# abstractqqq/polars_ds_extension

Hardware: AMD Instinct MI355X
Metric: grouped lstsq regressions/sec (1e8 rows x 16 f64 feats; Gram-build GB/s under gram_build) (higher is better)
Workload: dtype f64; 1 GPU; group_by(key).agg(lin_reg): 1000000 groups x 100 rows x 16 f64 feats of the frame (1e+08 rows), OLS with rank gate (pl_lr default path), inputs resident in HBM; `value`: the groups given as row offsets (pre-segmented, as Polars hands groups to pl_lr -- the cpu_baseline gets the same); the same step starting from a sorted int64 key column: grouped_by_key; groups_total=1000000, groups_per_gpu=1000000, rows_per_group=100, features=16, parallelism=group-sharded x1

## Files before the change

polars_ds_extension_amd/_lib.py:

```python
from __future__ import annotations

import ctypes as C
from pathlib import Path

_HERE = Path(__file__).resolve().parent
LIB_PATH = _HERE / "csrc" / "libpds_lstsq_hip.so"

PDS_HOST, PDS_DEVICE = 0, 1
SOLVERS = {"qr": 0, "svd": 1, "choleskey": 2}
SE_TYPES = {"se": 0, "hc0": 1, "hc1": 2, "hc2": 3, "hc3": 4}
WITHIN_SE_TYPES = {"se": 0, "cluster": 5, "cluster0": 6}
CLUSTER_SE_TYPES = {"cluster": 5, "cluster0": 6}
GLM_ROBUST_SE_TYPES = {"hc0": 1, "hc1": 2, "hc2": 3, "hc3": 4, "cluster": 5, "cluster0": 6}
PDS_REPORT_DERIVE_YVAR = 0x100

EXPORTS = [
    "pds_last_error", "pds_version", "pds_ctx_create", "pds_ctx_destroy", "pds_ctx_set_stream",
    "pds_ctx_synchronize", "pds_ctx_num_cus", "pds_ctx_set_option", "pds_ctx_get_option", "pds_grouped_fused_split", "pds_set_host_staging", "pds_rows_to_cols_f64", "pds_rows_to_cols_f32", "pds_glm_irls_f64", "pds_glm_irls_f32", "pds_glm_irls_grouped_f64", "pds_glm_irls_grouped_f32", "pds_glm_irls_by_key_f64", "pds_glm_irls_by_key_f32",
    "pds_glm_irls_wo_f64", "pds_glm_irls_wo_f32", "pds_glm_irls_wo_grouped_f64", "pds_glm_irls_wo_grouped_f32", "pds_glm_irls_wo_by_key_f64", "pds_glm_irls_wo_by_key_f32",
    "pds_glm_enet_f64", "pds_glm_enet_f32", "pds_glm_enet_grouped_f64", "pds_glm_enet_grouped_f32", "pds_glm_enet_by_key_f64", "pds_glm_enet_by_key_f32",
    "pds_glm_report_wo_grouped_f64", "pds_glm_report_wo_grouped_f32", "pds_glm_report_wo_by_key_f64", "pds_glm_report_wo_by_key_f32",
    "pds_glm_report_grouped_f64", "pds_glm_report_grouped_f32", "pds_glm_report_by_key_f64", "pds_glm_report_by_key_f32",
    "pds_glm_report_robust_f64", "pds_glm_report_robust_f32", "pds_glm_report_cluster_grouped_f64", "pds_glm_report_cluster_grouped_f32",
    "pds_glm_report_cluster_by_key_f64", "pds_glm_report_cluster_by_key_f32",
# ... 21 lines not shown
    "pds_lr_grouped_f64", "pds_lr_grouped_f32",
    "pds_rolling_lr_f64", "pds_rolling_lr_f32", "pds_recursive_lr_f64", "pds_recursive_lr_f32",
    "pds_recursive_lr_seeded_f64", "pds_recursive_lr_seeded_f32",
    "pds_rolling_lr_grouped_f64", "pds_rolling_lr_grouped_f32", "pds_recursive_lr_grouped_f64", "pds_recursive_lr_grouped_f32",
    "pds_rolling_lr_by_key_f64", "pds_rolling_lr_by_key_f32", "pds_recursive_lr_by_key_f64", "pds_recursive_lr_by_key_f32",
    "pds_lin_reg_report_nullable_f64", "pds_lin_reg_report_nullable_f32",
    "pds_lr_grouped_nullable_f64", "pds_lr_grouped_nullable_f32",
    "pds_lr_by_key_f64", "pds_lr_by_key_f32", "pds_lr_by_key_multi_f64", "pds_lr_by_key_multi_f32", "pds_lr_by_key_pred_multi_f64", "pds_lr_by_key_pred_multi_f32", "pds_host_alloc", "pds_host_free", "pds_device_count", "pds_device_alloc", "pds_device_free", "pds_ipc_export", "pds_ipc_open", "pds_ipc_close", "pds_signal_post", "pds_signal_wait", "pds_signal_wait_status", "pds_lr_grouped_pred_f64", "pds_lr_grouped_pred_f32", "pds_lr_by_key_pred_f64", "pds_lr_by_key_pred_f32", "pds_lr_grouped_weighted_f64", "pds_lr_grouped_weighted_f32",
    "pds_lr_with_inv_f64", "pds_lr_with_inv_f32",
    "pds_moments_f64", "pds_moments_f32", "pds_lr_from_moments_f64", "pds_lr_from_moments_f32",
    "pds_student_t_sf", "pds_student_t_ppf",
    "pds_allreduce_sum_f64", "pds_allreduce_sum_f32", "pds_scatter_rows_f64", "pds_scatter_rows_f32", "pds_gather_f64", "pds_gather_f32",
]


class LRParams(C.Structure):

    _fields_ = [
        ("add_bias", C.c_int),
        ("l1_reg", C.c_double),
        ("l2_reg", C.c_double),
        ("tol", C.c_double),
        ("solver", C.c_int),
        ("positive", C.c_int),
        ("max_iter", C.c_int),
        ("singular_x_tol", C.c_double),
    ]


class ReportF64(C.Structure):
    _fields_ = [(k, C.c_void_p) for k in ("beta", "std_err", "t", "p", "ci_lower", "ci_upper")] + [
        ("r2", C.c_double),
        ("adj_r2", C.c_double),
    ]


class ReportF32(C.Structure):
    _fields_ = [(k, C.c_void_p) for k in ("beta", "std_err", "t", "p", "ci_lower", "ci_upper")] + [
        ("r2", C.c_float),
        ("adj_r2", C.c_float),
    ]


class ReportGrouped(C.Structure):
    _fields_ = [(k, C.c_void_p) for k in ("beta", "std_err", "t", "p", "ci_lower", "ci_upper", "r2", "adj_r2", "is_null")]


class GlmReportOut(C.Structure):
    _fields_ = [(k, C.c_void_p) for k in ("std_err", "z", "p", "ci_lower", "ci_upper", "cov", "deviance", "null_deviance", "pearson_chi2",
                                          "dispersion", "df_resid", "report_null")]


class WithinOut(C.Structure):
    _fields_ = [("alpha", C.c_void_p), ("pred", C.c_void_p), ("resid", C.c_void_p), ("r2_overall", C.c_double),
                ("n_groups_used", C.c_int64), ("df_resid", C.c_int64)]


class GlmWithinOut(C.Structure):
    _fields_ = [(k, C.c_double * 16) for k in ("beta", "std_err", "z", "p", "ci_lower", "ci_upper")] + [
        ("cov", C.c_double * 256), ("deviance", C.c_double), ("pearson_chi2", C.c_double), ("dispersion", C.c_double),
        ("n_groups_used", C.c_int64), ("n_groups_dropped", C.c_int64), ("n_rows_used", C.c_int64), ("df_resid", C.c_int64),
        ("n_iter", C.c_int32), ("converged", C.c_int32), ("alpha", C.c_void_p), ("pred", C.c_void_p)]


class Within2Out(C.Structure):
    _fields_ = [("pred", C.c_void_p), ("resid", C.c_void_p), ("r2_overall", C.c_double), ("df_resid", C.c_int64),
                ("n_groups_used", C.c_int64), ("n_groups2_used", C.c_int64), ("n_components", C.c_int64), ("n_iter", C.c_int64)]


class Within2Effects(C.Structure):
    _fields_ = [("effects1", C.c_void_p), ("effects2", C.c_void_p), ("component1", C.c_void_p), ("component2", C.c_void_p),
                ("keys1", C.c_void_p), ("cap1", C.c_int64), ("n_graph_rounds", C.c_int64)]


class ClusterKey(C.Structure):
    _fields_ = [("codes", C.c_void_p), ("n_levels", C.c_int64), ("n_clusters", C.c_int64), ("nested1", C.c_int32), ("nested2", C.c_int32)]


class PdsError(RuntimeError):
    def __init__(self, code: int, msg: str):
        super().__init__(f"[pds {code}] {msg}")
        self.code = code
        self.msg = msg


_lib = None


def load() -> C.CDLL:
    global _lib
    if _lib is None:
        if not LIB_PATH.exists():
            raise ImportError(
                f"{LIB_PATH} is missing: run `python -c 'import __graft_entry__ as g; g.build()'` "
                "(hipcc --offload-arch=gfx950).  There is no CPU fallback."
            )
        try:
            import torch
        except Exception:
            pass
        lib = C.CDLL(str(LIB_PATH))
        lib.pds_last_error.restype = C.c_char_p
        lib.pds_version.restype = C.c_char_p
        lib.pds_student_t_sf.restype = C.c_double
        lib.pds_student_t_sf.argtypes = [C.c_double, C.c_double]
        lib.pds_student_t_ppf.restype = C.c_double
        lib.pds_student_t_ppf.argtypes = [C.c_double, C.c_double]
        lib.pds_ctx_create.argtypes = [C.c_int, C.POINTER(C.c_void_p)]
        lib.pds_ctx_destroy.argtypes = [C.c_void_p]
        lib.pds_ctx_destroy.restype = None
        lib.pds_ctx_set_stream.argtypes = [C.c_void_p, C.c_void_p]
        lib.pds_ctx_synchronize.argtypes = [C.c_void_p]
        lib.pds_ctx_num_cus.argtypes = [C.c_void_p]
        lib.pds_ctx_set_option.argtypes = [C.c_void_p, C.c_char_p, C.c_longlong]
        if hasattr(lib, "pds_ctx_get_option"):
            lib.pds_ctx_get_option.argtypes = [C.c_void_p, C.c_char_p, C.POINTER(C.c_longlong)]
        if hasattr(lib, "pds_set_host_staging"):
            lib.pds_set_host_staging.argtypes = [C.c_double, C.c_double]
        if hasattr(lib, "pds_ctx_workspace_spills"):
            lib.pds_ctx_workspace_spills.argtypes = [C.c_void_p]
            lib.pds_ctx_workspace_spills.restype = C.c_longlong
        for sfx, real in (("f64", C.c_double), ("f32", C.c_float)):
            if hasattr(lib, "pds_lr_multi_grouped_" + sfx):
                getattr(lib, "pds_lr_multi_grouped_" + sfx).argtypes = [C.c_void_p, C.c_void_p, C.c_int, C.c_int, C.c_int64, C.c_void_p,
                                                                      C.c_int64, C.c_int, C.c_int, real, C.c_int, real] + [C.c_void_p] * 5
                getattr(lib, "pds_lr_multi_by_key_" + sfx).argtypes = [C.c_void_p, C.c_void_p, C.c_void_p, C.c_int, C.c_int, C.c_int64, C.c_int,
                                                                     C.c_int, real, C.c_int, real, C.c_int64] + [C.c_void_p] * 7
            if hasattr(lib, "pds_lin_reg_within_grouped_" + sfx):
                getattr(lib, "pds_lin_reg_within_grouped_" + sfx).argtypes = [C.c_void_p, C.c_void_p, C.c_int, C.c_int64, C.c_void_p, C.c_int64,
                                                                            C.c_int, C.c_int, C.c_void_p, C.c_void_p]
                getattr(lib, "pds_lin_reg_within_by_key_" + sfx).argtypes = [C.c_void_p, C.c_void_p, C.c_void_p, C.c_int, C.c_int64, C.c_int, C.c_int,
                                                                           C.c_int64, C.c_void_p, C.c_void_p, C.c_void_p, C.c_void_p]
            if hasattr(lib, "pds_lin_reg_within2_grouped_" + sfx):
                getattr(lib, "pds_lin_reg_within2_grouped_" + sfx).argtypes = [C.c_void_p, C.c_void_p, C.c_int, C.c_int64, C.c_void_p, C.c_int64,
                                                                             C.c_void_p, C.c_int64, C.c_int, C.c_int, C.c_double, C.c_int,
                                                                             C.c_void_p, C.c_void_p]
                getattr(lib, "pds_lin_reg_within2_by_key_" + sfx).argtypes = [C.c_void_p, C.c_void_p, C.c_void_p, C.c_void_p, C.c_int64, C.c_int,
                                                                            C.c_int64, C.c_int, C.c_int, C.c_double, C.c_int, C.c_void_p,
                                                                            C.c_void_p, C.c_void_p]
            if hasattr(lib, "pds_lin_reg_within2_fx_grouped_" + sfx):
                getattr(lib, "pds_lin_reg_within2_fx_grouped_" + sfx).argtypes = getattr(lib, "pds_lin_reg_within2_grouped_" + sfx).argtypes + [C.c_void_p]
                getattr(lib, "pds_lin_reg_within2_fx_by_key_" + sfx).argtypes = getattr(lib, "pds_lin_reg_within2_by_key_" + sfx).argtypes + [C.c_void_p]
            if hasattr(lib, "pds_lin_reg_within_cl_grouped_" + sfx):
                for form in ("grouped_", "by_key_"):
                    getattr(lib, "pds_lin_reg_within_cl_" + form + sfx).argtypes = getattr(lib, "pds_lin_reg_within_" + form + sfx).argtypes + [C.c_void_p]
                    getattr(lib, "pds_lin_reg_within2_cl_" + form + sfx).argtypes = getattr(lib, "pds_lin_reg_within2_fx_" + form + sfx).argtypes + [C.c_void_p]
            if hasattr(lib, "pds_glm_within_grouped_" + sfx):
                getattr(lib, "pds_glm_within_grouped_" + sfx).argtypes = [C.c_void_p] * 4 + [C.c_int, C.c_int64, C.c_void_p, C.c_int64, C.c_int,
                                                                                             C.c_int, C.c_int, real, C.c_int, C.c_int, C.c_void_p]
                getattr(lib, "pds_glm_within_by_key_" + sfx).argtypes = [C.c_void_p] * 5 + [C.c_int, C.c_int64, C.c_int, C.c_int, C.c_int, real,
                                                                                            C.c_int, C.c_int, C.c_int64] + [C.c_void_p] * 3
        if hasattr(lib, "pds_absorb_components_i32"):
            lib.pds_absorb_components_i32.argtypes = [C.c_void_p, C.c_void_p, C.c_int64, C.c_void_p, C.c_int64, C.c_int64, C.c_int] + [C.c_void_p] * 6
        if hasattr(lib, "pds_ctx_workspace_bytes"):
            lib.pds_ctx_workspace_bytes.argtypes = [C.c_void_p, C.c_int]
            lib.pds_ctx_workspace_bytes.restype = C.c_longlong
        _lib = lib
    return _lib


def check(rc: int) -> None:
    if rc != 0:
        raise PdsError(rc, load().pds_last_error().decode("utf-8", "replace"))


def missing_exports() -> list[str]:
    lib = load()
    return [s for s in EXPORTS if not hasattr(lib, s)]
```

polars_ds_extension_amd/csrc/capi.hip:

```cpp
#include <algorithm>
#include <atomic>
#include <condition_variable>
#include <mutex>
#include <thread>
#include <chrono>
#include <cstdio>
#include <cstdlib>
#include <mutex>

#include <hipcub/hipcub.hpp>

#include "common.hpp"
#include "grouped_report.hpp"
#include "grouped_split_dev.hpp"

namespace pds {

#include "capi_core.hpp"
#include "capi_staging.hpp"
#include "capi_lr.hpp"
#include "capi_report.hpp"
#include "capi_staged_out.hpp"
#include "capi_keyed_frame.hpp"
#include "capi_group_chunks.hpp"
#include "capi_grouped.hpp"
#include "capi_report_grouped.hpp"
#include "capi_multi.hpp"
#include "capi_rolling.hpp"
#include "capi_models.hpp"
#include "capi_glm_grouped.hpp"
#include "capi_glm_report.hpp"
#include "capi_rcond_grouped.hpp"
#include "capi_multi_grouped.hpp"
#include "capi_mixed.hpp"
#include "capi_report_cluster.hpp"
#include "capi_within_cluster.hpp"
#include "capi_within.hpp"
#include "capi_within2.hpp"
#include "capi_glm_sandwich.hpp"
#include "capi_glm_within.hpp"

}

using namespace pds;

template <typename F>
static int with_cluster_key(pds_cluster_key* cl, pds_space space, F&& call) {
    if (!cl) return call(nullptr);
    pds::WithinCluster wc;
    wc.codes = cl->codes;
    wc.code_space = space;
    wc.n_levels = cl->n_levels;
    const int rc = call(&wc);
    cl->n_clusters = wc.n_clusters;
    cl->nested1 = wc.nested1;
    cl->nested2 = wc.nested2;
    return rc;
}

extern "C" {

const char* pds_last_error(void) { return g_err.c_str(); }
const char* pds_version(void) { return "pds_lstsq_hip 0.1.0 (gfx950)"; }

int pds_ctx_create(int device, pds_ctx** out) {
    if (!out) return fail(PDS_ERR_INVALID, "null out pointer");
    int ndev = 0;
    PDS_HIP_CHECK(hipGetDeviceCount(&ndev));
    if (device < 0 || device >= ndev) return fail(PDS_ERR_HIP, "no such HIP device");
    hipDeviceProp_t prop;
    PDS_HIP_CHECK(hipGetDeviceProperties(&prop, device));
    if (std::string(prop.gcnArchName).rfind("gfx950", 0) != 0)
        return fail(PDS_ERR_HIP, std::string("libpds_lstsq_hip is built for gfx950 only, device is ") + prop.gcnArchName);
    PDS_HIP_CHECK(hipSetDevice(device));
    pds_ctx* c = new pds_ctx();
    c->device = device;
    c->num_cus = prop.multiProcessorCount;
    if (hipStreamCreateWithFlags(&c->stream, hipStreamNonBlocking) != hipSuccess) {
        delete c;
        return fail(PDS_ERR_HIP, "hipStreamCreate failed");
    }
    c->own_stream = true;
    {
        const char* ks = std::getenv("PDS_KEYED_SORT");
        c->opt_keyed_sort = ks && ks[0] == '1';
        const char* wn = std::getenv("PDS_WIDE_F32_NATIVE");
        c->opt_wide_f32_native = wn && wn[0] == '1';
    }
    const size_t pbytes = (size_t)c->num_cus * 8 * kPartStride * sizeof(double);
    if (hipMalloc(reinterpret_cast<void**>(&c->partials), pbytes) != hipSuccess) {
        (void)hipStreamDestroy(c->stream);
        delete c;
        return fail(PDS_ERR_HIP, "hipMalloc(partials) failed");
    }
    *out = c;
    return PDS_OK;
}

void pds_ctx_destroy(pds_ctx* ctx) {
    if (!ctx) return;
    (void)hipSetDevice(ctx->device);
    (void)hipStreamSynchronize(ctx->stream);
    if (ctx->partials) (void)hipFree(ctx->partials);
    if (ctx->ws.ptr) (void)hipFree(ctx->ws.ptr);
    for (void* q : ctx->ws_spill) (void)hipFree(q);
    if (ctx->stage.ptr) (void)hipFree(ctx->stage.ptr);
    if (ctx->solve_ws.ptr) (void)hipFree(ctx->solve_ws.ptr);
    if (ctx->keyed.ptr) (void)hipFree(ctx->keyed.ptr);
    if (ctx->wkeyed.ptr) (void)hipFree(ctx->wkeyed.ptr);
    if (ctx->mark_count) (void)hipFree(ctx->mark_count);
    if (ctx->wait_timeouts) (void)hipFree(ctx->wait_timeouts);
    if (ctx->mark_host) (void)hipHostFree(ctx->mark_host);
    if (ctx->pinned) (void)hipHostFree(ctx->pinned);
    if (ctx->pinned_in) (void)hipHostFree(ctx->pinned_in);
    for (auto& e : ctx->ev_pending) {
        (void)hipEventDestroy(e.a);
        (void)hipEventDestroy(e.b);
    }
    for (auto e : ctx->ev_pool) (void)hipEventDestroy(e);
    if (ctx->own_stream && ctx->stream) (void)hipStreamDestroy(ctx->stream);
    delete ctx;
}

int pds_ctx_set_stream(pds_ctx* ctx, void* hip_stream) {
    if (!ctx) return fail(PDS_ERR_INVALID, "null ctx");
    PDS_HIP_CHECK(hipSetDevice(ctx->device));
    PDS_HIP_CHECK(hipStreamSynchronize(ctx->stream));
    if (ctx->own_stream && ctx->stream) (void)hipStreamDestroy(ctx->stream);
    ctx->stream = reinterpret_cast<hipStream_t>(hip_stream);
    ctx->own_stream = false;
    return PDS_OK;
}

int pds_ctx_synchronize(pds_ctx* ctx) {
    if (!ctx) return fail(PDS_ERR_INVALID, "null ctx");
    PDS_HIP_CHECK(hipStreamSynchronize(ctx->stream));
    return PDS_OK;
}

int pds_ctx_num_cus(const pds_ctx* ctx) { return ctx ? ctx->num_cus : 0; }

int pds_ctx_set_option(pds_ctx* ctx, const char* name, long long value) {
    if (!ctx || !name) return fail(PDS_ERR_INVALID, "null argument");
    const std::string n(name);
    if (n == "keyed_sort") ctx->opt_keyed_sort = value != 0;
    else if (n == "wide_f32_native") ctx->opt_wide_f32_native = value != 0;
    else if (n == "glm_split_rows") ctx->opt_glm_split_rows = value > 0 ? (int64_t)value : 0;
    else if (n == "mixed_split_rows") ctx->opt_mixed_split_rows = value > 0 ? (int64_t)value : 0;
    else if (n == "cluster_split_rows") ctx->opt_cluster_split_rows = value > 0 ? (int64_t)value : 0;
    else if (n == "cluster_waves") ctx->opt_cluster_waves = value > 0 ? (int64_t)value : 0;
    else if (n == "within_split_rows") ctx->opt_within_split_rows = value > 0 ? (int64_t)value : 0;
    else if (n == "within2_accel") {
        if (value != 0 && value != 1) return fail(PDS_ERR_INVALID, "within2_accel: 0 (plain sweeps) or 1 (Irons-Tuck)");
        ctx->opt_within2_accel = (int64_t)value;
    } else if (n == "report_chunk_groups") ctx->opt_report_chunk_groups = value > 0 ? (int64_t)value : 0;
    else if (n == "grouped_fused_waves") ctx->opt_fused_waves = value > 0 ? (int64_t)value : 0;
    else if (n == "grouped_fused_late_permille") {
        if (value < 0 || value > 999) return fail(PDS_ERR_INVALID, "grouped_fused_late_permille: 0 (the default rule) or 1 .. 999");
        ctx->opt_fused_late_permille = (int64_t)value;
    } else if (n == "grouped_multi_route") {
        if (value < 0 || value > 2) return fail(PDS_ERR_INVALID, "grouped_multi_route: 0 (choose), 1 (one kernel) or 2 (per target)");
        ctx->opt_multi_route = (int64_t)value;
    } else if (n == "grouped_multi_waves") ctx->opt_multi_waves = value > 0 ? (int64_t)value : 0;
    else if (n == "rolling_waves") ctx->opt_rolling_waves = value > 0 ? (int64_t)value : 0;
    else return fail(PDS_ERR_INVALID, "unknown context option: " + n);
    return PDS_OK;
}

int pds_ctx_get_option(const pds_ctx* ctx, const char* name, long long* value) {
    if (!ctx || !name || !value) return fail(PDS_ERR_INVALID, "null argument");
    const std::string n(name);
    if (n == "keyed_sort") *value = ctx->opt_keyed_sort ? 1 : 0;
    else if (n == "wide_f32_native") *value = ctx->opt_wide_f32_native ? 1 : 0;
    else if (n == "glm_split_rows") *value = ctx->opt_glm_split_rows;
    else if (n == "mixed_split_rows") *value = ctx->opt_mixed_split_rows;
    else if (n == "cluster_split_rows") *value = ctx->opt_cluster_split_rows;
    else if (n == "cluster_waves") *value = ctx->opt_cluster_waves;
    else if (n == "within_split_rows") *value = ctx->opt_within_split_rows;
    else if (n == "within2_accel") *value = ctx->opt_within2_accel;
    else if (n == "report_chunk_groups") *value = ctx->opt_report_chunk_groups;
    else if (n == "grouped_fused_waves") *value = ctx->opt_fused_waves;
    else if (n == "grouped_fused_late_permille") *value = ctx->opt_fused_late_permille;
    else if (n == "grouped_multi_route") *value = ctx->opt_multi_route;
    else if (n == "grouped_multi_waves") *value = ctx->opt_multi_waves;
    else if (n == "rolling_waves") *value = ctx->opt_rolling_waves;
    else return fail(PDS_ERR_INVALID, "unknown context option: " + n);
    return PDS_OK;
}

int pds_grouped_fused_split(const int64_t* group_offsets, int64_t n_groups, int waves, int late_permille, int64_t* first_group,
                            int64_t* end_group) {
    if (!group_offsets || !first_group || !end_group) return fail(PDS_ERR_INVALID, "null argument");
    if (n_groups < 0 || waves < 1 || late_permille < 0 || late_permille > 999) return fail(PDS_ERR_INVALID, "pds_grouped_fused_split: bad argument");
    const int64_t base = group_offsets[0], total = group_offsets[n_groups] - base;
    auto bound = [&](int64_t w) -> int64_t {
        if (w == 0) return 0;
        if (w == waves) return n_groups;
        return std::lower_bound(group_offsets, group_offsets + n_groups, base + pds::fused_split_row(w, waves, total, late_permille)) - group_offsets;
    };
    for (int w = 0; w < waves; ++w) {
        first_group[w] = bound(w);
        end_group[w] = std::max(bound(w + 1), first_group[w]);
    }
    return PDS_OK;
}

int pds_glm_irls_f64(pds_ctx* ctx, const double* const* cols, int n_feat, int64_t n_rows, pds_space space, int add_bias, int link,
                     int variance, double tol, int max_iter, double* coeffs, int* n_iter) {
    return pds::glm_irls_impl<double>(ctx, cols, n_feat, n_rows, space, add_bias, link, variance, tol, max_iter, coeffs, n_iter);
}
int pds_glm_irls_f32(pds_ctx* ctx, const float* const* cols, int n_feat, int64_t n_rows, pds_space space, int add_bias, int link,
                     int variance, float tol, int max_iter, float* coeffs, int* n_iter) {
    return pds::glm_irls_impl<float>(ctx, cols, n_feat, n_rows, space, add_bias, link, variance, tol, max_iter, coeffs, n_iter);
}

int pds_glm_irls_grouped_f64(pds_ctx* ctx, const double* const* cols, int n_feat, int64_t n_rows, const int64_t* group_offsets,
                             int64_t n_groups, pds_space space, int add_bias, int link, int variance, double tol, int max_iter,
                             double* coeffs, int32_t* n_iter, uint8_t* is_null, double* pred, uint8_t* row_null) {
    return pds::glm_grouped_impl<double>(ctx, cols, n_feat, n_rows, group_offsets, n_groups, space, add_bias, link, variance, 0.0, 0.0, tol,
                                         max_iter, coeffs, n_iter, is_null, pred, row_null);
}
int pds_glm_irls_grouped_f32(pds_ctx* ctx, const float* const* cols, int n_feat, int64_t n_rows, const int64_t* group_offsets,
                             int64_t n_groups, pds_space space, int add_bias, int link, int variance, float tol, int max_iter,
                             float* coeffs, int32_t* n_iter, uint8_t* is_null, float* pred, uint8_t* row_null) {
    return pds::glm_grouped_impl<float>(ctx, cols, n_feat, n_rows, group_offsets, n_groups, space, add_bias, link, variance, 0.0f, 0.0f, tol,
                                        max_iter, coeffs, n_iter, is_null, pred, row_null);
}
int pds_glm_irls_by_key_f64(pds_ctx* ctx, const double* const* cols, const int64_t* keys, int n_feat, int64_t n_rows, pds_space space,
                            int add_bias, int link, int variance, double tol, int max_iter, int64_t max_groups, int64_t* out_keys,
                            double* coeffs, int32_t* n_iter, uint8_t* is_null, int64_t* n_groups, double* pred, uint8_t* row_null) {
    return pds::glm_by_key_impl<double>(ctx, cols, keys, n_feat, n_rows, space, add_bias, link, variance, 0.0, 0.0, tol, max_iter, max_groups,
                                        out_keys, coeffs, n_iter, is_null, n_groups, pred, row_null);
}
int pds_glm_irls_by_key_f32(pds_ctx* ctx, const float* const* cols, const int64_t* keys, int n_feat, int64_t n_rows, pds_space space,
                            int add_bias, int link, int variance, float tol, int max_iter, int64_t max_groups, int64_t* out_keys,
                            float* coeffs, int32_t* n_iter, uint8_t* is_null, int64_t* n_groups, float* pred, uint8_t* row_null) {
    return pds::glm_by_key_impl<float>(ctx, cols, keys, n_feat, n_rows, space, add_bias, link, variance, 0.0f, 0.0f, tol, max_iter, max_groups,
                                       out_keys, coeffs, n_iter, is_null, n_groups, pred, row_null);
}

int pds_glm_irls_wo_f64(pds_ctx* ctx, const double* const* cols, const double* weights, const double* offset, int n_feat, int64_t n_rows,
                        pds_space space, int add_bias, int link, int variance, double tol, int max_iter, double* coeffs, int* n_iter) {
    return pds::glm_irls_wo_impl<double>(ctx, cols, weights, offset, n_feat, n_rows, space, add_bias, link, variance, tol, max_iter, coeffs,
                                         n_iter);
}
int pds_glm_irls_wo_f32(pds_ctx* ctx, const float* const* cols, const float* weights, const float* offset, int n_feat, int64_t n_rows,
                        pds_space space, int add_bias, int link, int variance, float tol, int max_iter, float* coeffs, int* n_iter) {
    return pds::glm_irls_wo_impl<float>(ctx, cols, weights, offset, n_feat, n_rows, space, add_bias, link, variance, tol, max_iter, coeffs,
                                        n_iter);
}
int pds_glm_irls_wo_grouped_f64(pds_ctx* ctx, const double* const* cols, const double* weights, const double* offset, int n_feat,
                                int64_t n_rows, const int64_t* group_offsets, int64_t n_groups, pds_space space, int add_bias, int link,
                                int variance, double tol, int max_iter, double* coeffs, int32_t* n_iter, uint8_t* is_null, double* pred,
                                uint8_t* row_null) {
    return pds::glm_grouped_impl<double>(ctx, cols, n_feat, n_rows, group_offsets, n_groups, space, add_bias, link, variance, 0.0, 0.0, tol,
                                         max_iter, coeffs, n_iter, is_null, pred, row_null, nullptr, weights, offset);
}
int pds_glm_irls_wo_grouped_f32(pds_ctx* ctx, const float* const* cols, const float* weights, const float* offset, int n_feat, int64_t n_rows,
                                const int64_t* group_offsets, int64_t n_groups, pds_space space, int add_bias, int link, int variance,
                                float tol, int max_iter, float* coeffs, int32_t* n_iter, uint8_t* is_null, float* pred, uint8_t* row_null) {
    return pds::glm_grouped_impl<float>(ctx, cols, n_feat, n_rows, group_offsets, n_groups, space, add_bias, link, variance, 0.0f, 0.0f, tol,
                                        max_iter, coeffs, n_iter, is_null, pred, row_null, nullptr, weights, offset);
}
int pds_glm_irls_wo_by_key_f64(pds_ctx* ctx, const double* const* cols, const double* weights, const double* offset, const int64_t* keys,
                               int n_feat, int64_t n_rows, pds_space space, int add_bias, int link, int variance, double tol, int max_iter,
                               int64_t max_groups, int64_t* out_keys, double* coeffs, int32_t* n_iter, uint8_t* is_null, int64_t* n_groups,
                               double* pred, uint8_t* row_null) {
    return pds::glm_by_key_impl<double>(ctx, cols, keys, n_feat, n_rows, space, add_bias, link, variance, 0.0, 0.0, tol, max_iter, max_groups,
                                        out_keys, coeffs, n_iter, is_null, n_groups, pred, row_null, weights, offset);
}
int pds_glm_irls_wo_by_key_f32(pds_ctx* ctx, const float* const* cols, const float* weights, const float* offset, const int64_t* keys,
                               int n_feat, int64_t n_rows, pds_space space, int add_bias, int link, int variance, float tol, int max_iter,
                               int64_t max_groups, int64_t* out_keys, float* coeffs, int32_t* n_iter, uint8_t* is_null, int64_t* n_groups,
                               float* pred, uint8_t* row_null) {
    return pds::glm_by_key_impl<float>(ctx, cols, keys, n_feat, n_rows, space, add_bias, link, variance, 0.0f, 0.0f, tol, max_iter, max_groups,
                                       out_keys, coeffs, n_iter, is_null, n_groups, pred, row_null, weights, offset);
}

int pds_glm_report_grouped_f64(pds_ctx* ctx, const double* const* cols, int n_feat, int64_t n_rows, const int64_t* group_offsets,
                               int64_t n_groups, pds_space space, int add_bias, int link, int variance, double tol, int max_iter,
                               double* coeffs, int32_t* n_iter, uint8_t* is_null, const pds_glm_report_out* out) {
    return pds::glm_report_grouped_impl<double>(ctx, cols, n_feat, n_rows, group_offsets, n_groups, space, add_bias, link, variance, tol,
                                                max_iter, coeffs, n_iter, is_null, out);
}
int pds_glm_report_grouped_f32(pds_ctx* ctx, const float* const* cols, int n_feat, int64_t n_rows, const int64_t* group_offsets,
                               int64_t n_groups, pds_space space, int add_bias, int link, int variance, float tol, int max_iter,
                               float* coeffs, int32_t* n_iter, uint8_t* is_null, const pds_glm_report_out* out) {
    return pds::glm_report_grouped_impl<float>(ctx, cols, n_feat, n_rows, group_offsets, n_groups, space, add_bias, link, variance, tol,
                                               max_iter, coeffs, n_iter, is_null, out);
}
int pds_glm_report_by_key_f64(pds_ctx* ctx, const double* const* cols, const int64_t* keys, int n_feat, int64_t n_rows, pds_space space,
                              int add_bias, int link, int variance, double tol, int max_iter, int64_t max_groups, int64_t* out_keys,
                              double* coeffs, int32_t* n_iter, uint8_t* is_null, int64_t* n_groups, const pds_glm_report_out* out) {
    return pds::glm_report_by_key_impl<double>(ctx, cols, keys, n_feat, n_rows, space, add_bias, link, variance, tol, max_iter, max_groups,
                                               out_keys, coeffs, n_iter, is_null, n_groups, out);
}
int pds_glm_report_by_key_f32(pds_ctx* ctx, const float* const* cols, const int64_t* keys, int n_feat, int64_t n_rows, pds_space space,
                              int add_bias, int link, int variance, float tol, int max_iter, int64_t max_groups, int64_t* out_keys,
                              float* coeffs, int32_t* n_iter, uint8_t* is_null, int64_t* n_groups, const pds_glm_report_out* out) {
    return pds::glm_report_by_key_impl<float>(ctx, cols, keys, n_feat, n_rows, space, add_bias, link, variance, tol, max_iter, max_groups,
                                              out_keys, coeffs, n_iter, is_null, n_groups, out);
}

int pds_glm_report_wo_grouped_f64(pds_ctx* ctx, const double* const* cols, const double* weights, const double* offset, int n_feat, int64_t n_rows,
                                  const int64_t* group_offsets, int64_t n_groups, pds_space space, int add_bias, int link, int variance,
                                  double tol, int max_iter, double* coeffs, int32_t* n_iter, uint8_t* is_null, const pds_glm_report_out* out) {
    return pds::glm_report_grouped_impl<double>(ctx, cols, n_feat, n_rows, group_offsets, n_groups, space, add_bias, link, variance, tol,
                                                max_iter, coeffs, n_iter, is_null, out, weights, offset);
}
int pds_glm_report_wo_by_key_f64(pds_ctx* ctx, const double* const* cols, const double* weights, const double* offset, const int64_t* keys, int n_feat,
                                 int64_t n_rows, pds_space space, int add_bias, int link, int variance, double tol, int max_iter,
                                 int64_t max_groups, int64_t* out_keys, double* coeffs, int32_t* n_iter, uint8_t* is_null, int64_t* n_groups,
                                 const pds_glm_report_out* out) {
    return pds::glm_report_by_key_impl<double>(ctx, cols, keys, n_feat, n_rows, space, add_bias, link, variance, tol, max_iter, max_groups,
                                               out_keys, coeffs, n_iter, is_null, n_groups, out, weights, offset);
}
int pds_glm_report_wo_grouped_f32(pds_ctx* ctx, const float* const* cols, const float* weights, const float* offset, int n_feat, int64_t n_rows,
                                  const int64_t* group_offsets, int64_t n_groups, pds_space space, int add_bias, int link, int variance,
                                  float tol, int max_iter, float* coeffs, int32_t* n_iter, uint8_t* is_null, const pds_glm_report_out* out) {
    return pds::glm_report_grouped_impl<float>(ctx, cols, n_feat, n_rows, group_offsets, n_groups, space, add_bias, link, variance, tol,
                                                max_iter, coeffs, n_iter, is_null, out, weights, offset);
}
int pds_glm_report_wo_by_key_f32(pds_ctx* ctx, const float* const* cols, const float* weights, const float* offset, const int64_t* keys, int n_feat,
                                 int64_t n_rows, pds_space space, int add_bias, int link, int variance, float tol, int max_iter,
                                 int64_t max_groups, int64_t* out_keys, float* coeffs, int32_t* n_iter, uint8_t* is_null, int64_t* n_groups,
                                 const pds_glm_report_out* out) {
    return pds::glm_report_by_key_impl<float>(ctx, cols, keys, n_feat, n_rows, space, add_bias, link, variance, tol, max_iter, max_groups,
                                               out_keys, coeffs, n_iter, is_null, n_groups, out, weights, offset);
}

int pds_glm_report_robust_f64(pds_ctx* ctx, const double* const* cols, const double* weights, const double* offset, int n_feat, int64_t n_rows,
                              pds_space space, int add_bias, int link, int variance, double tol, int max_iter, int se_type, double* coeffs,
                              int32_t* n_iter, const pds_glm_report_out* out, int64_t* n_clusters) {
    return pds::glm_sandwich_impl<double>(ctx, cols, weights, offset, n_feat, n_rows, nullptr, 0, space, add_bias, link, variance, tol, max_iter,
                                       se_type, false, coeffs, n_iter, out, n_clusters);
}
int pds_glm_report_cluster_grouped_f64(pds_ctx* ctx, const double* const* cols, const double* weights, const double* offset, int n_feat,
                                       int64_t n_rows, const int64_t* cluster_offsets, int64_t n_offsets, pds_space space, int add_bias,
// ... 371 lines not shown
                                                absorb_tol, absorb_max_iter, out, extra);
}
int pds_lin_reg_within2_grouped_f32(pds_ctx* ctx, const float* const* cols, int n_feat, int64_t n_rows, const int64_t* group_offsets,
                                    int64_t n_groups, const int32_t* codes2, int64_t n_levels2, pds_space space, int se_type,
                                    double absorb_tol, int absorb_max_iter, pds_report_f32* out, pds_within2_out* extra) {
    return within2_impl<float, pds_report_f32>(ctx, cols, n_feat, n_rows, group_offsets, n_groups, space, codes2, space, n_levels2, space, se_type,
                                               absorb_tol, absorb_max_iter, out, extra);
}
int pds_lin_reg_within2_by_key_f64(pds_ctx* ctx, const double* const* cols, const int64_t* keys, const int32_t* codes2, int64_t n_levels2,
                                   int n_feat, int64_t n_rows, pds_space space, int se_type, double absorb_tol, int absorb_max_iter,
                                   pds_report_f64* out, pds_within2_out* extra, int64_t* n_groups) {
    return within2_by_key_impl<double, pds_report_f64>(ctx, cols, keys, codes2, n_levels2, n_feat, n_rows, space, se_type, absorb_tol,
                                                       absorb_max_iter, out, extra, n_groups);
}
int pds_lin_reg_within2_by_key_f32(pds_ctx* ctx, const float* const* cols, const int64_t* keys, const int32_t* codes2, int64_t n_levels2,
                                   int n_feat, int64_t n_rows, pds_space space, int se_type, double absorb_tol, int absorb_max_iter,
                                   pds_report_f32* out, pds_within2_out* extra, int64_t* n_groups) {
    return within2_by_key_impl<float, pds_report_f32>(ctx, cols, keys, codes2, n_levels2, n_feat, n_rows, space, se_type, absorb_tol,
                                                      absorb_max_iter, out, extra, n_groups);
}
int pds_lin_reg_within2_fx_grouped_f64(pds_ctx* ctx, const double* const* cols, int n_feat, int64_t n_rows, const int64_t* group_offsets,
                                       int64_t n_groups, const int32_t* codes2, int64_t n_levels2, pds_space space, int se_type,
                                       double absorb_tol, int absorb_max_iter, pds_report_f64* out, pds_within2_out* extra,
                                       pds_within2_effects* fx) {
    return within2_impl<double, pds_report_f64>(ctx, cols, n_feat, n_rows, group_offsets, n_groups, space, codes2, space, n_levels2, space, se_type,
                                                absorb_tol, absorb_max_iter, out, extra, nullptr, fx);
}
int pds_lin_reg_within2_fx_grouped_f32(pds_ctx* ctx, const float* const* cols, int n_feat, int64_t n_rows, const int64_t* group_offsets,
                                       int64_t n_groups, const int32_t* codes2, int64_t n_levels2, pds_space space, int se_type,
                                       double absorb_tol, int absorb_max_iter, pds_report_f32* out, pds_within2_out* extra,
                                       pds_within2_effects* fx) {
    return within2_impl<float, pds_report_f32>(ctx, cols, n_feat, n_rows, group_offsets, n_groups, space, codes2, space, n_levels2, space, se_type,
                                               absorb_tol, absorb_max_iter, out, extra, nullptr, fx);
}
int pds_lin_reg_within2_fx_by_key_f64(pds_ctx* ctx, const double* const* cols, const int64_t* keys, const int32_t* codes2, int64_t n_levels2,
                                      int n_feat, int64_t n_rows, pds_space space, int se_type, double absorb_tol, int absorb_max_iter,
                                      pds_report_f64* out, pds_within2_out* extra, int64_t* n_groups, pds_within2_effects* fx) {
    return within2_by_key_impl<double, pds_report_f64>(ctx, cols, keys, codes2, n_levels2, n_feat, n_rows, space, se_type, absorb_tol,
                                                       absorb_max_iter, out, extra, n_groups, fx);
}
int pds_lin_reg_within2_fx_by_key_f32(pds_ctx* ctx, const float* const* cols, const int64_t* keys, const int32_t* codes2, int64_t n_levels2,
                                      int n_feat, int64_t n_rows, pds_space space, int se_type, double absorb_tol, int absorb_max_iter,
                                      pds_report_f32* out, pds_within2_out* extra, int64_t* n_groups, pds_within2_effects* fx) {
    return within2_by_key_impl<float, pds_report_f32>(ctx, cols, keys, codes2, n_levels2, n_feat, n_rows, space, se_type, absorb_tol,
                                                      absorb_max_iter, out, extra, n_groups, fx);
}
int pds_lin_reg_within_cl_grouped_f64(pds_ctx* ctx, const double* const* cols, int n_feat, int64_t n_rows, const int64_t* group_offsets,
                                      int64_t n_groups, pds_space space, int se_type, pds_report_f64* out, pds_within_out* extra, pds_cluster_key* cl) {
    return with_cluster_key(cl, space, [&](WithinCluster* wc) {
        return within_impl<double, pds_report_f64>(ctx, cols, n_feat, n_rows, group_offsets, n_groups, space, space, se_type, out, extra, nullptr, nullptr, wc);
    });
}
int pds_lin_reg_within_cl_by_key_f64(pds_ctx* ctx, const double* const* cols, const int64_t* keys, int n_feat, int64_t n_rows, pds_space space,
                                     int se_type, int64_t max_groups, int64_t* out_keys, pds_report_f64* out, pds_within_out* extra, int64_t* n_groups,
                                     pds_cluster_key* cl) {
    return with_cluster_key(cl, space, [&](WithinCluster* wc) {
        return within_by_key_impl<double, pds_report_f64>(ctx, cols, keys, n_feat, n_rows, space, se_type, max_groups, out_keys, out, extra, n_groups, wc);
    });
}
int pds_lin_reg_within2_cl_grouped_f64(pds_ctx* ctx, const double* const* cols, int n_feat, int64_t n_rows, const int64_t* group_offsets,
                                       int64_t n_groups, const int32_t* codes2, int64_t n_levels2, pds_space space, int se_type,
                                       double absorb_tol, int absorb_max_iter, pds_report_f64* out, pds_within2_out* extra, pds_within2_effects* fx,
                                       pds_cluster_key* cl) {
    return with_cluster_key(cl, space, [&](WithinCluster* wc) {
        return within2_impl<double, pds_report_f64>(ctx, cols, n_feat, n_rows, group_offsets, n_groups, space, codes2, space, n_levels2, space, se_type, absorb_tol,
                                        absorb_max_iter, out, extra, nullptr, fx, wc);
    });
}
int pds_lin_reg_within2_cl_by_key_f64(pds_ctx* ctx, const double* const* cols, const int64_t* keys, const int32_t* codes2, int64_t n_levels2,
                                      int n_feat, int64_t n_rows, pds_space space, int se_type, double absorb_tol, int absorb_max_iter,
                                      pds_report_f64* out, pds_within2_out* extra, int64_t* n_groups, pds_within2_effects* fx, pds_cluster_key* cl) {
    return with_cluster_key(cl, space, [&](WithinCluster* wc) {
        return within2_by_key_impl<double, pds_report_f64>(ctx, cols, keys, codes2, n_levels2, n_feat, n_rows, space, se_type, absorb_tol, absorb_max_iter, out,
                                               extra, n_groups, fx, wc);
    });
}
int pds_lin_reg_within_cl_grouped_f32(pds_ctx* ctx, const float* const* cols, int n_feat, int64_t n_rows, const int64_t* group_offsets,
                                      int64_t n_groups, pds_space space, int se_type, pds_report_f32* out, pds_within_out* extra, pds_cluster_key* cl) {
    return with_cluster_key(cl, space, [&](WithinCluster* wc) {
        return within_impl<float, pds_report_f32>(ctx, cols, n_feat, n_rows, group_offsets, n_groups, space, space, se_type, out, extra, nullptr, nullptr, wc);
    });
}
int pds_lin_reg_within_cl_by_key_f32(pds_ctx* ctx, const float* const* cols, const int64_t* keys, int n_feat, int64_t n_rows, pds_space space,
                                     int se_type, int64_t max_groups, int64_t* out_keys, pds_report_f32* out, pds_within_out* extra, int64_t* n_groups,
                                     pds_cluster_key* cl) {
    return with_cluster_key(cl, space, [&](WithinCluster* wc) {
        return within_by_key_impl<float, pds_report_f32>(ctx, cols, keys, n_feat, n_rows, space, se_type, max_groups, out_keys, out, extra, n_groups, wc);
    });
}
int pds_lin_reg_within2_cl_grouped_f32(pds_ctx* ctx, const float* const* cols, int n_feat, int64_t n_rows, const int64_t* group_offsets,
                                       int64_t n_groups, const int32_t* codes2, int64_t n_levels2, pds_space space, int se_type,
                                       double absorb_tol, int absorb_max_iter, pds_report_f32* out, pds_within2_out* extra, pds_within2_effects* fx,
                                       pds_cluster_key* cl) {
    return with_cluster_key(cl, space, [&](WithinCluster* wc) {
        return within2_impl<float, pds_report_f32>(ctx, cols, n_feat, n_rows, group_offsets, n_groups, space, codes2, space, n_levels2, space, se_type, absorb_tol,
                                        absorb_max_iter, out, extra, nullptr, fx, wc);
    });
}
int pds_lin_reg_within2_cl_by_key_f32(pds_ctx* ctx, const float* const* cols, const int64_t* keys, const int32_t* codes2, int64_t n_levels2,
                                      int n_feat, int64_t n_rows, pds_space space, int se_type, double absorb_tol, int absorb_max_iter,
                                      pds_report_f32* out, pds_within2_out* extra, int64_t* n_groups, pds_within2_effects* fx, pds_cluster_key* cl) {
    return with_cluster_key(cl, space, [&](WithinCluster* wc) {
        return within2_by_key_impl<float, pds_report_f32>(ctx, cols, keys, codes2, n_levels2, n_feat, n_rows, space, se_type, absorb_tol, absorb_max_iter, out,
                                               extra, n_groups, fx, wc);
    });
}
int pds_absorb_components_i32(pds_ctx* ctx, const int32_t* codes1, int64_t n_levels1, const int32_t* codes2, int64_t n_levels2, int64_t n_rows,
                              pds_space space, int32_t* component1, int32_t* component2, int64_t* n1, int64_t* n2, int64_t* n_components,
                              int* n_rounds) {
    return absorb_components_impl(ctx, codes1, n_levels1, codes2, n_levels2, n_rows, space, component1, component2, n1, n2, n_components, n_rounds);
}

int pds_report_fit_from_moments_f64(pds_ctx* ctx, const double* moments, int n_feat, int add_bias, double* beta, double* inv) {
    return report_fit_impl<double>(ctx, moments, n_feat, add_bias, beta, inv);
}
int pds_report_fit_from_moments_f32(pds_ctx* ctx, const float* moments, int n_feat, int add_bias, float* beta, float* inv) {
    return report_fit_impl<float>(ctx, moments, n_feat, add_bias, beta, inv);
}
int pds_report_partials_f64(pds_ctx* ctx, const double* const* cols, const double* weights, int n_feat, int64_t n_rows,
                            pds_space space, int add_bias, int se_type, const double* beta, const double* inv, double* partials) {
    return report_partials_impl<double>(ctx, cols, weights, n_feat, n_rows, space, add_bias, se_type, beta, inv, partials);
}
int pds_report_partials_f32(pds_ctx* ctx, const float* const* cols, const float* weights, int n_feat, int64_t n_rows,
                            pds_space space, int add_bias, int se_type, const float* beta, const float* inv, double* partials) {
    return report_partials_impl<float>(ctx, cols, weights, n_feat, n_rows, space, add_bias, se_type, beta, inv, partials);
}
int pds_report_finish_f64(int n_feat, int add_bias, int se_type, int weighted, int64_t n_rows_total, double y_var,
                          const double* beta, const double* inv, const double* partials, pds_report_f64* out) {
    return report_finish_impl<double, pds_report_f64>(n_feat, add_bias, se_type, weighted, n_rows_total, y_var, beta, inv, partials, out);
}
int pds_report_finish_f32(int n_feat, int add_bias, int se_type, int weighted, int64_t n_rows_total, float y_var,
                          const float* beta, const float* inv, const double* partials, pds_report_f32* out) {
    return report_finish_impl<float, pds_report_f32>(n_feat, add_bias, se_type, weighted, n_rows_total, y_var, beta, inv, partials, out);
}

int pds_lin_reg_report_nullable_f64(pds_ctx* ctx, const double* const* cols, const uint8_t* const* validity,
                                    const int64_t* bit_offsets, int n_feat, int64_t n_rows, pds_space space, int null_policy,
                                    double fill_value, int add_bias, int se_type, double y_var, pds_report_f64* out,
                                    int64_t* n_used) {
    return report_impl<double, pds_report_f64>(ctx, cols, nullptr, n_feat, n_rows, space, add_bias, se_type, y_var, out, true,
                                               validity, bit_offsets, null_policy, fill_value, n_used);
}
int pds_lin_reg_report_nullable_f32(pds_ctx* ctx, const float* const* cols, const uint8_t* const* validity,
                                    const int64_t* bit_offsets, int n_feat, int64_t n_rows, pds_space space, int null_policy,
                                    float fill_value, int add_bias, int se_type, float y_var, pds_report_f32* out,
                                    int64_t* n_used) {
    return report_impl<float, pds_report_f32>(ctx, cols, nullptr, n_feat, n_rows, space, add_bias, se_type, y_var, out, true,
                                              validity, bit_offsets, null_policy, fill_value, n_used);
}

int pds_lr_grouped_f64(pds_ctx* ctx, const double* const* cols, int n_feat, int64_t n_rows,
                       const int64_t* group_offsets, int64_t n_groups, pds_space space, const pds_lr_params* prm,
                       double* coeffs, uint8_t* is_null) {
    return grouped_impl<double>(ctx, cols, n_feat, n_rows, group_offsets, n_groups, space, prm, coeffs, is_null);
}
int pds_lr_grouped_f32(pds_ctx* ctx, const float* const* cols, int n_feat, int64_t n_rows,
                       const int64_t* group_offsets, int64_t n_groups, pds_space space, const pds_lr_params* prm,
                       float* coeffs, uint8_t* is_null) {
    return grouped_impl<float>(ctx, cols, n_feat, n_rows, group_offsets, n_groups, space, prm, coeffs, is_null);
}

int pds_lr_grouped_nullable_f64(pds_ctx* ctx, const double* const* cols, const uint8_t* const* validity,
                                const int64_t* bit_offsets, int n_feat, int64_t n_rows, const int64_t* group_offsets,
                                int64_t n_groups, pds_space space, int null_policy, double fill_value, const pds_lr_params* prm,
                                double* coeffs, uint8_t* is_null) {
    return grouped_impl<double>(ctx, cols, n_feat, n_rows, group_offsets, n_groups, space, prm, coeffs, is_null, true, validity,
                                bit_offsets, null_policy, fill_value);
}
int pds_lr_grouped_nullable_f32(pds_ctx* ctx, const float* const* cols, const uint8_t* const* validity,
                                const int64_t* bit_offsets, int n_feat, int64_t n_rows, const int64_t* group_offsets,
                                int64_t n_groups, pds_space space, int null_policy, float fill_value, const pds_lr_params* prm,
                                float* coeffs, uint8_t* is_null) {
    return grouped_impl<float>(ctx, cols, n_feat, n_rows, group_offsets, n_groups, space, prm, coeffs, is_null, true, validity,
                               bit_offsets, null_policy, fill_value);
}

int pds_lr_with_inv_f64(pds_ctx* ctx, const double* const* cols, int n_feat, int64_t n_rows, pds_space space, int add_bias,
                        double lambda, double* coeffs, double* inv) {
    return pds::lr_with_inv_impl<double>(ctx, cols, n_feat, n_rows, space, add_bias, lambda, coeffs, inv);
}
int pds_lr_with_inv_f32(pds_ctx* ctx, const float* const* cols, int n_feat, int64_t n_rows, pds_space space, int add_bias,
                        float lambda, float* coeffs, float* inv) {
    return pds::lr_with_inv_impl<float>(ctx, cols, n_feat, n_rows, space, add_bias, (double)lambda, coeffs, inv);
}

int pds_lr_grouped_weighted_f64(pds_ctx* ctx, const double* const* cols, const double* weights, int n_feat, int64_t n_rows,
                                const int64_t* group_offsets, int64_t n_groups, pds_space space, const pds_lr_params* prm,
                                double* coeffs, uint8_t* is_null) {
    return pds::grouped_weighted_impl<double>(ctx, cols, weights, n_feat, n_rows, group_offsets, n_groups, space, prm, coeffs, is_null);
}
int pds_lr_grouped_weighted_f32(pds_ctx* ctx, const float* const* cols, const float* weights, int n_feat, int64_t n_rows,
                                const int64_t* group_offsets, int64_t n_groups, pds_space space, const pds_lr_params* prm,
                                float* coeffs, uint8_t* is_null) {
    return pds::grouped_weighted_impl<float>(ctx, cols, weights, n_feat, n_rows, group_offsets, n_groups, space, prm, coeffs, is_null);
}

int pds_lr_by_key_multi_f64(pds_ctx* const* ctxs, int n_ctx, int n_slices, const double* const* cols, const int64_t* keys, int n_feat,
                            int64_t n_rows, const pds_lr_params* prm, int64_t max_groups, int64_t* out_keys, double* coeffs,
                            uint8_t* is_null, int64_t* n_groups) {
    return pds::lr_by_key_multi_impl<double>(ctxs, n_ctx, n_slices, cols, keys, n_feat, n_rows, prm, max_groups, out_keys, coeffs, is_null,
                                             n_groups);
}
int pds_lr_by_key_multi_f32(pds_ctx* const* ctxs, int n_ctx, int n_slices, const float* const* cols, const int64_t* keys, int n_feat,
                            int64_t n_rows, const pds_lr_params* prm, int64_t max_groups, int64_t* out_keys, float* coeffs,
                            uint8_t* is_null, int64_t* n_groups) {
    return pds::lr_by_key_multi_impl<float>(ctxs, n_ctx, n_slices, cols, keys, n_feat, n_rows, prm, max_groups, out_keys, coeffs, is_null,
                                            n_groups);
}
int pds_lr_by_key_pred_multi_f64(pds_ctx* const* ctxs, int n_ctx, int n_slices, const double* const* cols, const double* weights,
                                 const int64_t* keys, int n_feat, int64_t n_rows, const pds_lr_params* prm, double* pred, double* resid,
                                 uint8_t* row_null) {
    return pds::lr_by_key_pred_multi_impl<double>(ctxs, n_ctx, n_slices, cols, weights, keys, n_feat, n_rows, prm, pred, resid, row_null);
}
int pds_lr_by_key_pred_multi_f32(pds_ctx* const* ctxs, int n_ctx, int n_slices, const float* const* cols, const float* weights,
                                 const int64_t* keys, int n_feat, int64_t n_rows, const pds_lr_params* prm, float* pred, float* resid,
                                 uint8_t* row_null) {
    return pds::lr_by_key_pred_multi_impl<float>(ctxs, n_ctx, n_slices, cols, weights, keys, n_feat, n_rows, prm, pred, resid, row_null);
}
int pds_host_alloc(size_t bytes, void** out) {
    if (!out) return pds::fail(PDS_ERR_INVALID, "null argument");
    *out = nullptr;
    PDS_HIP_CHECK(hipHostMalloc(out, bytes ? bytes : 1, hipHostMallocPortable));
    return PDS_OK;
}
int pds_host_free(void* p) {
    if (p) PDS_HIP_CHECK(hipHostFree(p));
    return PDS_OK;
}
int pds_device_count(int* n) {
    if (!n) return pds::fail(PDS_ERR_INVALID, "null argument");
    *n = 0;
    PDS_HIP_CHECK(hipGetDeviceCount(n));
    return PDS_OK;
}
static_assert(sizeof(hipIpcMemHandle_t) == PDS_IPC_HANDLE_BYTES, "the handle travels as 64 opaque bytes");
int pds_device_alloc(int device, size_t bytes, int fine_grained, void** out) {
    if (!out) return pds::fail(PDS_ERR_INVALID, "null argument");
    *out = nullptr;
    PDS_HIP_CHECK(hipSetDevice(device));
    if (fine_grained) PDS_HIP_CHECK(hipExtMallocWithFlags(out, bytes ? bytes : 1, hipDeviceMallocFinegrained));
    else PDS_HIP_CHECK(hipMalloc(out, bytes ? bytes : 1));
    return PDS_OK;
}
namespace pds {
__global__ void signal_post_kernel(unsigned* word, unsigned value) {
    __hip_atomic_store(word, value, __ATOMIC_RELEASE, __HIP_MEMORY_SCOPE_SYSTEM);
}
__global__ __launch_bounds__(64) void signal_wait_kernel(const unsigned* words, int n, unsigned value, long long budget_ticks, int* timed_out) {
    const int lane = threadIdx.x;
    const long long t0 = wall_clock64();
    bool ok = lane >= n;
    while (!__all(ok)) {
        if (!ok) ok = (int)(__hip_atomic_load(words + lane, __ATOMIC_ACQUIRE, __HIP_MEMORY_SCOPE_SYSTEM) - value) >= 0;
        if (wall_clock64() - t0 > budget_ticks) {
            if (lane == 0) atomicAdd(timed_out, 1);
            break;
        }
        __builtin_amdgcn_s_sleep(8);
    }
}
}
int pds_signal_post(pds_ctx* ctx, unsigned* word, unsigned value) {
    if (!ctx || !word) return pds::fail(PDS_ERR_INVALID, "null argument");
    PDS_HIP_CHECK(hipSetDevice(ctx->device));
    hipLaunchKernelGGL(pds::signal_post_kernel, dim3(1), dim3(1), 0, ctx->stream, word, value);
    PDS_HIP_CHECK(hipGetLastError());
    return PDS_OK;
}
int pds_signal_wait(pds_ctx* ctx, const unsigned* words, int n_words, unsigned value, int timeout_ms) {
    if (!ctx || !words || n_words < 0 || n_words > 64) return pds::fail(PDS_ERR_INVALID, "pds_signal_wait: up to 64 words");
    if (n_words == 0) return PDS_OK;
    PDS_HIP_CHECK(hipSetDevice(ctx->device));
    if (!ctx->wait_timeouts) {
        PDS_HIP_CHECK(hipMalloc(reinterpret_cast<void**>(&ctx->wait_timeouts), 64));
        PDS_HIP_CHECK(hipMemsetAsync(ctx->wait_timeouts, 0, 64, ctx->stream));
    }
    int rate_khz = 100000;
    (void)hipDeviceGetAttribute(&rate_khz, hipDeviceAttributeWallClockRate, ctx->device);
    const long long budget = (long long)(timeout_ms > 0 ? timeout_ms : 2000) * (long long)rate_khz;
    hipLaunchKernelGGL(pds::signal_wait_kernel, dim3(1), dim3(64), 0, ctx->stream, words, n_words, value, budget,
                       ctx->wait_timeouts);
    PDS_HIP_CHECK(hipGetLastError());
    return PDS_OK;
}
int pds_signal_wait_status(pds_ctx* ctx, int* timed_out) {
    if (!ctx || !timed_out) return pds::fail(PDS_ERR_INVALID, "null argument");
    *timed_out = 0;
    if (!ctx->wait_timeouts) return PDS_OK;
    PDS_HIP_CHECK(hipSetDevice(ctx->device));
    PDS_HIP_CHECK(hipMemcpyAsync(timed_out, ctx->wait_timeouts, sizeof(int), hipMemcpyDeviceToHost, ctx->stream));
    PDS_HIP_CHECK(hipStreamSynchronize(ctx->stream));
    return PDS_OK;
}
int pds_device_free(int device, void* p) {
    if (!p) return PDS_OK;
    PDS_HIP_CHECK(hipSetDevice(device));
    PDS_HIP_CHECK(hipFree(p));
    return PDS_OK;
}
int pds_ipc_export(int device, void* p, unsigned char* handle) {
    if (!p || !handle) return pds::fail(PDS_ERR_INVALID, "null argument");
    PDS_HIP_CHECK(hipSetDevice(device));
    hipIpcMemHandle_t h;
    PDS_HIP_CHECK(hipIpcGetMemHandle(&h, p));
    std::memcpy(handle, &h, sizeof(h));
    return PDS_OK;
}
int pds_ipc_open(int device, const unsigned char* handle, void** mapped) {
    if (!handle || !mapped) return pds::fail(PDS_ERR_INVALID, "null argument");
    *mapped = nullptr;
    PDS_HIP_CHECK(hipSetDevice(device));
    hipIpcMemHandle_t h;
// ... 68 lines not shown
int pds_wls_report_grouped_f64(pds_ctx* ctx, const double* const* cols, const double* weights, int n_feat, int64_t n_rows,
                               const int64_t* group_offsets, int64_t n_groups, pds_space space, int add_bias, const double* y_var,
                               pds_report_grouped_f64* out) {
    if (!weights) return pds::fail(PDS_ERR_INVALID, "null argument");
    return pds::report_grouped_impl<double>(ctx, cols, weights, n_feat, n_rows, group_offsets, n_groups, space, add_bias, PDS_SE, y_var,
                                            reinterpret_cast<const pds::ReportGroupedOut<double>*>(out));
}
int pds_wls_report_by_key_f64(pds_ctx* ctx, const double* const* cols, const double* weights, const int64_t* keys, int n_feat,
                              int64_t n_rows, pds_space space, int add_bias, int64_t max_groups, int64_t* out_keys,
                              pds_report_grouped_f64* out, int64_t* n_groups) {
    if (!weights) return pds::fail(PDS_ERR_INVALID, "null argument");
    return pds::report_by_key_impl<double>(ctx, cols, weights, keys, n_feat, n_rows, space, add_bias, PDS_SE, max_groups, out_keys,
                                           reinterpret_cast<const pds::ReportGroupedOut<double>*>(out), n_groups);
}
int pds_wls_report_grouped_f32(pds_ctx* ctx, const float* const* cols, const float* weights, int n_feat, int64_t n_rows,
                               const int64_t* group_offsets, int64_t n_groups, pds_space space, int add_bias, const float* y_var,
                               pds_report_grouped_f32* out) {
    if (!weights) return pds::fail(PDS_ERR_INVALID, "null argument");
    return pds::report_grouped_impl<float>(ctx, cols, weights, n_feat, n_rows, group_offsets, n_groups, space, add_bias, PDS_SE, y_var,
                                            reinterpret_cast<const pds::ReportGroupedOut<float>*>(out));
}
int pds_wls_report_by_key_f32(pds_ctx* ctx, const float* const* cols, const float* weights, const int64_t* keys, int n_feat,
                              int64_t n_rows, pds_space space, int add_bias, int64_t max_groups, int64_t* out_keys,
                              pds_report_grouped_f32* out, int64_t* n_groups) {
    if (!weights) return pds::fail(PDS_ERR_INVALID, "null argument");
    return pds::report_by_key_impl<float>(ctx, cols, weights, keys, n_feat, n_rows, space, add_bias, PDS_SE, max_groups, out_keys,
                                           reinterpret_cast<const pds::ReportGroupedOut<float>*>(out), n_groups);
}
int pds_student_t_sf_device(pds_ctx* ctx, const double* x, const double* df, int64_t n, double* out) {
    return pds::student_t_sf_device_impl(ctx, x, df, n, out);
}
int pds_lr_by_key_f64(pds_ctx* ctx, const double* const* cols, const int64_t* keys, int n_feat, int64_t n_rows, pds_space space,
                      const pds_lr_params* prm, int64_t max_groups, int64_t* out_keys, double* coeffs, uint8_t* is_null,
                      int64_t* n_groups) {
    return pds::lr_by_key_impl<double>(ctx, cols, keys, n_feat, n_rows, space, prm, max_groups, out_keys, coeffs, is_null, n_groups);
}
int pds_lr_by_key_f32(pds_ctx* ctx, const float* const* cols, const int64_t* keys, int n_feat, int64_t n_rows, pds_space space,
                      const pds_lr_params* prm, int64_t max_groups, int64_t* out_keys, float* coeffs, uint8_t* is_null,
                      int64_t* n_groups) {
    return pds::lr_by_key_impl<float>(ctx, cols, keys, n_feat, n_rows, space, prm, max_groups, out_keys, coeffs, is_null, n_groups);
}

int pds_rolling_lr_f64(pds_ctx* ctx, const double* const* cols, int n_feat, int64_t n_rows, pds_space space,
                       int add_bias, int64_t window, int64_t min_size, double lambda, double* coeffs, double* pred,
                       uint8_t* valid) {
    return rolling_impl<double>(ctx, cols, n_feat, n_rows, space, add_bias, window, min_size, lambda, false, coeffs, pred, valid);
}
int pds_rolling_lr_f32(pds_ctx* ctx, const float* const* cols, int n_feat, int64_t n_rows, pds_space space,
                       int add_bias, int64_t window, int64_t min_size, float lambda, float* coeffs, float* pred,
                       uint8_t* valid) {
    return rolling_impl<float>(ctx, cols, n_feat, n_rows, space, add_bias, window, min_size, lambda, false, coeffs, pred, valid);
}
int pds_recursive_lr_f64(pds_ctx* ctx, const double* const* cols, int n_feat, int64_t n_rows, pds_space space,
                         int add_bias, int64_t start_with, double lambda, double* coeffs, double* pred,
                         uint8_t* valid) {
    return rolling_impl<double>(ctx, cols, n_feat, n_rows, space, add_bias, start_with, 0, lambda, true, coeffs, pred, valid);
}
int pds_recursive_lr_f32(pds_ctx* ctx, const float* const* cols, int n_feat, int64_t n_rows, pds_space space,
                         int add_bias, int64_t start_with, float lambda, float* coeffs, float* pred, uint8_t* valid) {
    return rolling_impl<float>(ctx, cols, n_feat, n_rows, space, add_bias, start_with, 0, lambda, true, coeffs, pred, valid);
}

int pds_rolling_lr_grouped_f64(pds_ctx* ctx, const double* const* cols, int n_feat, int64_t n_rows, const int64_t* group_offsets,
                               int64_t n_groups, pds_space space, int add_bias, int64_t window, int64_t min_size, double lambda,
                               double* coeffs, double* pred, uint8_t* valid) {
    return rolling_grouped_impl<double>(ctx, cols, n_feat, n_rows, group_offsets, n_groups, space, add_bias, window, min_size, lambda, false,
                                        coeffs, pred, valid);
}
int pds_rolling_lr_grouped_f32(pds_ctx* ctx, const float* const* cols, int n_feat, int64_t n_rows, const int64_t* group_offsets,
                               int64_t n_groups, pds_space space, int add_bias, int64_t window, int64_t min_size, float lambda,
                               float* coeffs, float* pred, uint8_t* valid) {
    return rolling_grouped_impl<float>(ctx, cols, n_feat, n_rows, group_offsets, n_groups, space, add_bias, window, min_size, lambda, false,
                                       coeffs, pred, valid);
}
int pds_recursive_lr_grouped_f64(pds_ctx* ctx, const double* const* cols, int n_feat, int64_t n_rows, const int64_t* group_offsets,
                                 int64_t n_groups, pds_space space, int add_bias, int64_t start_with, double lambda, double* coeffs,
                                 double* pred, uint8_t* valid) {
    return rolling_grouped_impl<double>(ctx, cols, n_feat, n_rows, group_offsets, n_groups, space, add_bias, start_with, 0, lambda, true,
                                        coeffs, pred, valid);
}
int pds_recursive_lr_grouped_f32(pds_ctx* ctx, const float* const* cols, int n_feat, int64_t n_rows, const int64_t* group_offsets,
                                 int64_t n_groups, pds_space space, int add_bias, int64_t start_with, float lambda, float* coeffs,
                                 float* pred, uint8_t* valid) {
    return rolling_grouped_impl<float>(ctx, cols, n_feat, n_rows, group_offsets, n_groups, space, add_bias, start_with, 0, lambda, true,
                                       coeffs, pred, valid);
}
int pds_rolling_lr_by_key_f64(pds_ctx* ctx, const double* const* cols, const int64_t* keys, int n_feat, int64_t n_rows, pds_space space,
                              int add_bias, int64_t window, int64_t min_size, double lambda, double* coeffs, double* pred, uint8_t* valid) {
    return rolling_by_key_impl<double>(ctx, cols, keys, n_feat, n_rows, space, add_bias, window, min_size, lambda, false, coeffs, pred, valid);
}
int pds_rolling_lr_by_key_f32(pds_ctx* ctx, const float* const* cols, const int64_t* keys, int n_feat, int64_t n_rows, pds_space space,
                              int add_bias, int64_t window, int64_t min_size, float lambda, float* coeffs, float* pred, uint8_t* valid) {
    return rolling_by_key_impl<float>(ctx, cols, keys, n_feat, n_rows, space, add_bias, window, min_size, lambda, false, coeffs, pred, valid);
}
int pds_recursive_lr_by_key_f64(pds_ctx* ctx, const double* const* cols, const int64_t* keys, int n_feat, int64_t n_rows, pds_space space,
                                int add_bias, int64_t start_with, double lambda, double* coeffs, double* pred, uint8_t* valid) {
    return rolling_by_key_impl<double>(ctx, cols, keys, n_feat, n_rows, space, add_bias, start_with, 0, lambda, true, coeffs, pred, valid);
}
int pds_recursive_lr_by_key_f32(pds_ctx* ctx, const float* const* cols, const int64_t* keys, int n_feat, int64_t n_rows, pds_space space,
                                int add_bias, int64_t start_with, float lambda, float* coeffs, float* pred, uint8_t* valid) {
    return rolling_by_key_impl<float>(ctx, cols, keys, n_feat, n_rows, space, add_bias, start_with, 0, lambda, true, coeffs, pred, valid);
}

int pds_recursive_lr_seeded_f64(pds_ctx* ctx, const double* const* cols, int n_feat, int64_t n_rows, pds_space space,
                                int add_bias, int64_t start_with, double lambda, const double* seed_moments,
                                double* coeffs, double* pred, uint8_t* valid) {
    return rolling_impl<double>(ctx, cols, n_feat, n_rows, space, add_bias, start_with, 0, lambda, true, coeffs, pred, valid,
                                seed_moments);
}
int pds_recursive_lr_seeded_f32(pds_ctx* ctx, const float* const* cols, int n_feat, int64_t n_rows, pds_space space,
                                int add_bias, int64_t start_with, float lambda, const float* seed_moments, float* coeffs,
                                float* pred, uint8_t* valid) {
    return rolling_impl<float>(ctx, cols, n_feat, n_rows, space, add_bias, start_with, 0, lambda, true, coeffs, pred, valid,
                               seed_moments);
}

int pds_moments_f64(pds_ctx* ctx, const double* const* cols, const double* weights, int n_feat, int64_t n_rows,
                    pds_space space, double* moments, pds_space out_space) {
    return moments_impl<double>(ctx, cols, weights, n_feat, n_rows, space, moments, out_space);
}
int pds_moments_f32(pds_ctx* ctx, const float* const* cols, const float* weights, int n_feat, int64_t n_rows,
                    pds_space space, float* moments, pds_space out_space) {
    return moments_impl<float>(ctx, cols, weights, n_feat, n_rows, space, moments, out_space);
}
int pds_lr_from_moments_f64(pds_ctx* ctx, const double* moments, pds_space mom_space, int n_feat,
                            const pds_lr_params* prm, double* coeffs, int* is_null) {
    return from_moments_impl<double>(ctx, moments, mom_space, n_feat, prm, coeffs, is_null);
}
int pds_lr_from_moments_f32(pds_ctx* ctx, const float* moments, pds_space mom_space, int n_feat,
                            const pds_lr_params* prm, float* coeffs, int* is_null) {
    return from_moments_impl<float>(ctx, moments, mom_space, n_feat, prm, coeffs, is_null);
}

int pds_allreduce_sum_f64(pds_ctx* const* ctxs, int n_ctx, double* const* bufs, int64_t count, int prefix) {
    return pds::allreduce_sum_impl<double>(ctxs, n_ctx, bufs, count, prefix);
}
int pds_allreduce_sum_f32(pds_ctx* const* ctxs, int n_ctx, float* const* bufs, int64_t count, int prefix) {
    return pds::allreduce_sum_impl<float>(ctxs, n_ctx, bufs, count, prefix);
}
int pds_scatter_rows_f64(pds_ctx* const* ctxs, int n_ctx, const double* const* cols, int n_cols, const int64_t* bounds, double* const* const* dst) {
    return pds::scatter_rows_impl<double>(ctxs, n_ctx, cols, n_cols, bounds, dst);
}
int pds_scatter_rows_f32(pds_ctx* const* ctxs, int n_ctx, const float* const* cols, int n_cols, const int64_t* bounds, float* const* const* dst) {
    return pds::scatter_rows_impl<float>(ctxs, n_ctx, cols, n_cols, bounds, dst);
}
int pds_gather_f64(pds_ctx* const* ctxs, int n_ctx, const double* const* src, const int64_t* counts, double* dst) {
    return pds::gather_impl<double>(ctxs, n_ctx, src, counts, dst);
}
int pds_gather_f32(pds_ctx* const* ctxs, int n_ctx, const float* const* src, const int64_t* counts, float* dst) {
    return pds::gather_impl<float>(ctxs, n_ctx, src, counts, dst);
}
int pds_debug_last_multi_route(void) { return pds::g_multi_route; }
int pds_debug_last_grouped_route(void) { return pds::g_grouped_route; }
int pds_debug_last_by_key_route(int* info ) {
    if (info)
        for (int i = 0; i < 4; ++i) info[i] = pds::g_by_key_info[i];
    return pds::g_by_key_route;
}
}
```

polars_ds_extension_amd/csrc/capi_core.hpp:

```cpp
#pragma once

static thread_local std::string g_err;

struct StageTrace {
    pds_ctx* ctx;
    const char* what;
    bool on;
    std::chrono::steady_clock::time_point t0;
    StageTrace(pds_ctx* c, const char* w) : ctx(c), what(w) {
        static const bool env = [] { const char* e = std::getenv("PDS_TRACE"); return e && e[0] == '1'; }();
        on = env;
        if (on) t0 = std::chrono::steady_clock::now();
    }
    void mark(const char* stage) {
        if (!on) return;
        (void)hipStreamSynchronize(ctx->stream);
        const auto t1 = std::chrono::steady_clock::now();
        std::fprintf(stderr, "[pds trace] %s: %-28s %8.2f ms\n", what, stage, std::chrono::duration<double, std::milli>(t1 - t0).count());
        t0 = t1;
    }
};
void set_error(const std::string& msg) { g_err = msg; }
int fail(int code, const std::string& msg) {
    g_err = msg;
    return code;
}

static hipEvent_t take_event(pds_ctx* ctx) {
    if (!ctx->ev_pool.empty()) {
        hipEvent_t e = ctx->ev_pool.back();
        ctx->ev_pool.pop_back();
        return e;
    }
    hipEvent_t e = nullptr;
    if (hipEventCreate(&e) != hipSuccess) return nullptr;
    return e;
}
KernelTimer::KernelTimer(pds_ctx* c, int k) : ctx(c), kind(k) {
    if (!ctx->timing) return;
    a = take_event(ctx);
    b = take_event(ctx);
    if (a) (void)hipEventRecord(a, ctx->stream);
}
KernelTimer::~KernelTimer() {
    if (!ctx->timing || !a || !b) return;
    (void)hipEventRecord(b, ctx->stream);
    ctx->ev_pending.push_back({kind, a, b});
}

int ensure_ws(pds_ctx* ctx, Workspace& w, size_t bytes) {
    if (bytes <= w.bytes) return PDS_OK;
    if (w.ptr) {
        PDS_HIP_CHECK(hipStreamSynchronize(ctx->stream));
        PDS_HIP_CHECK(hipFree(w.ptr));
        w.ptr = nullptr;
        w.bytes = 0;
    }
    size_t want = std::max(bytes, (size_t)1 << 20);
    want = (want + ((size_t)1 << 20) - 1) & ~(((size_t)1 << 20) - 1);
    PDS_HIP_CHECK(hipMalloc(&w.ptr, want));
    w.bytes = want;
    return PDS_OK;
}

int ensure_pinned(pds_ctx* ctx, size_t bytes) {
    if (bytes <= ctx->pinned_bytes) return PDS_OK;
    if (ctx->pinned) {
        PDS_HIP_CHECK(hipStreamSynchronize(ctx->stream));
        PDS_HIP_CHECK(hipHostFree(ctx->pinned));
        ctx->pinned = nullptr;
        ctx->pinned_bytes = 0;
    }
    size_t want = std::max(bytes, (size_t)1 << 16);
    PDS_HIP_CHECK(hipHostMalloc(&ctx->pinned, want, hipHostMallocDefault));
    ctx->pinned_bytes = want;
    return PDS_OK;
}

int ws_reserve(pds_ctx* ctx, size_t total_bytes) {
    ctx->ws_used = 0;
    for (void* q : ctx->ws_spill) (void)hipFree(q);
    ctx->ws_spill.clear();
    return ensure_ws(ctx, ctx->ws, total_bytes + 4096);
}
void* ws_take(pds_ctx* ctx, size_t bytes) {
    const size_t off = (ctx->ws_used + 255) & ~(size_t)255;
    if (off + bytes > ctx->ws.bytes) {
        void* q = nullptr;
        ++ctx->ws_spill_count;
        if (hipMalloc(&q, bytes + 256) != hipSuccess) return nullptr;
        ctx->ws_spill.push_back(q);
        return q;
    }
    ctx->ws_used = off + bytes;
    return static_cast<char*>(ctx->ws.ptr) + off;
}

constexpr size_t kSmallFrameBytes = (size_t)1 << 20;

template <typename T>
int make_device_cols(pds_ctx* ctx, const T* const* cols, const T* weights, int n_feat, int64_t n_rows,
                     pds_space space, DeviceCols<T>& out) {
    const int nc = n_feat + 1 + (weights ? 1 : 0);
    out.nc = nc;
    out.h_ptrs.resize(nc);
    std::vector<const T*> src(nc);
    for (int c = 0; c < n_feat; ++c) src[c] = cols[c + 1];
    src[n_feat] = cols[0];
    if (weights) src[n_feat + 1] = weights;
    if (space == PDS_DEVICE) {
        for (int c = 0; c < nc; ++c) out.h_ptrs[c] = src[c];
    } else {
        const size_t col_bytes = ((size_t)n_rows * sizeof(T) + 255) & ~(size_t)255;
        const size_t tbl_entries = (size_t)std::max(nc, 18);
        const size_t tbl_bytes = (tbl_entries * sizeof(T*) + 255) & ~(size_t)255;
        if (tbl_bytes + col_bytes * nc <= kSmallFrameBytes) {
            const size_t total = tbl_bytes + col_bytes * nc;
            if (total > ctx->pinned_in_bytes) {
                if (ctx->pinned_in) {
                    PDS_HIP_CHECK(hipStreamSynchronize(ctx->stream));
                    PDS_HIP_CHECK(hipHostFree(ctx->pinned_in));
                    ctx->pinned_in = nullptr;
                    ctx->pinned_in_bytes = 0;
                }
                PDS_HIP_CHECK(hipHostMalloc(&ctx->pinned_in, kSmallFrameBytes, hipHostMallocDefault));
                ctx->pinned_in_bytes = kSmallFrameBytes;
            }
            if (int rc = ensure_ws(ctx, ctx->stage, total)) return rc;
            char* pin = static_cast<char*>(ctx->pinned_in);
            char* dev = static_cast<char*>(ctx->stage.ptr);
            for (int c = 0; c < nc; ++c) {
                std::memcpy(pin + tbl_bytes + col_bytes * c, src[c], (size_t)n_rows * sizeof(T));
                out.h_ptrs[c] = reinterpret_cast<const T*>(dev + tbl_bytes + col_bytes * c);
            }
            out.h_ptrs.resize(tbl_entries, out.h_ptrs[0]);
            std::memcpy(pin, out.h_ptrs.data(), tbl_entries * sizeof(T*));
            PDS_HIP_CHECK(hipMemcpyAsync(dev, pin, total, hipMemcpyHostToDevice, ctx->stream));
            out.d_ptrs = reinterpret_cast<const T**>(dev);
            return PDS_OK;
        }
        if (int rc = ensure_ws(ctx, ctx->stage, col_bytes * nc)) return rc;
        for (int c = 0; c < nc; ++c) {
            T* dst = reinterpret_cast<T*>(static_cast<char*>(ctx->stage.ptr) + col_bytes * c);
            PDS_HIP_CHECK(hipMemcpyAsync(dst, src[c], (size_t)n_rows * sizeof(T), hipMemcpyHostToDevice, ctx->stream));
            out.h_ptrs[c] = dst;
        }
    }
    out.h_ptrs.resize(std::max(nc, 18), out.h_ptrs[0]);
    out.d_ptrs = reinterpret_cast<const T**>(ws_take(ctx, sizeof(T*) * out.h_ptrs.size()));
    PDS_HIP_CHECK(hipMemcpyAsync(out.d_ptrs, out.h_ptrs.data(), sizeof(T*) * out.h_ptrs.size(), hipMemcpyHostToDevice, ctx->stream));
    return PDS_OK;
}
```

polars_ds_extension_amd/csrc/capi_grouped.hpp:

```cpp
#pragma once

static thread_local int g_grouped_route = 0;
static thread_local int g_by_key_route = -1;
static thread_local int g_by_key_info[4] = {0, 0, 0, 0};
__global__ void mark_small_groups_kernel(const int64_t* __restrict__ off, int64_t n_groups, int pp, uint8_t* __restrict__ flags) {
    const int64_t g = (int64_t)blockIdx.x * blockDim.x + threadIdx.x;
    if (g < n_groups && off[g + 1] - off[g] < pp) flags[g] = 1;
}
template <typename T>
__global__ void nan_flagged_kernel(const uint8_t* __restrict__ flags, int64_t n_groups, int pp, T* __restrict__ coeffs) {
    const int64_t i = (int64_t)blockIdx.x * blockDim.x + threadIdx.x;
    if (i < n_groups * pp && flags[i / pp]) coeffs[i] = (T)__builtin_nan("");
}

template <typename T>
static int grouped_big(pds_ctx* ctx, const DeviceCols<T>& dc, int n_feat, const int64_t* d_off, int64_t n_groups, int64_t chunk,
                       const Method& method, const pds_lr_params* prm, const SolveParams& sp, T* d_mom, T* d_coeffs,
                       uint8_t* d_null) {
    const int bias = prm->add_bias ? 1 : 0, pp = n_feat + bias, q = n_feat + 2, nc = n_feat + 1;
    std::vector<int64_t> off((size_t)n_groups + 1);
    PDS_HIP_CHECK(hipMemcpyAsync(off.data(), d_off, off.size() * 8, hipMemcpyDeviceToHost, ctx->stream));
    PDS_HIP_CHECK(hipStreamSynchronize(ctx->stream));
    std::vector<const T*> tables((size_t)n_groups * nc);
    for (int64_t g = 0; g < n_groups; ++g)
        for (int c = 0; c < nc; ++c) tables[(size_t)g * nc + c] = dc.h_ptrs[c] + off[g];
    const T** d_tables = reinterpret_cast<const T**>(ws_take(ctx, tables.size() * sizeof(T*)));
    PDS_HIP_CHECK(hipMemcpyAsync(d_tables, tables.data(), tables.size() * sizeof(T*), hipMemcpyHostToDevice, ctx->stream));
    PDS_HIP_CHECK(hipStreamSynchronize(ctx->stream));
    const bool f32 = sizeof(T) == 4;
    for (int64_t g0 = 0; g0 < n_groups; g0 += chunk) {
        const int64_t gc = std::min(chunk, n_groups - g0);
        for (int64_t g = g0; g < g0 + gc; ++g) {
            T* rec = d_mom + (size_t)(g - g0) * q * q;
            const int64_t ng = off[g + 1] - off[g];
            if (ng <= 0) {
                PDS_HIP_CHECK(hipMemsetAsync(rec, 0, sizeof(T) * (size_t)q * q, ctx->stream));
                continue;
            }
            DeviceCols<T> dg;
            dg.nc = nc;
            dg.d_ptrs = d_tables + (size_t)g * nc;
            dg.h_ptrs.assign(tables.begin() + (size_t)g * nc, tables.begin() + (size_t)(g + 1) * nc);
            const size_t mark = ctx->ws_used;
            const int rc = launch_moments_wide<T>(ctx, dg, n_feat, ng, false, rec);
            ctx->ws_used = mark;
            if (rc) return rc;
        }
        T* co = d_coeffs + g0 * pp;
        uint8_t* fl = d_null + g0;
        if (method.kind == Method::OLS) {
            if (int rc = launch_solve<T>(ctx, d_mom, gc, sp, co, fl, nullptr, nullptr)) return rc;
            hipLaunchKernelGGL(mark_small_groups_kernel, dim3((unsigned)((gc + 255) / 256)), dim3(256), 0, ctx->stream, d_off + g0, gc,
                               pp, fl);
            hipLaunchKernelGGL((nan_flagged_kernel<T>), dim3((unsigned)((gc * pp + 255) / 256)), dim3(256), 0, ctx->stream, fl, gc, pp,
                               co);
            PDS_HIP_CHECK(hipGetLastError());
        } else if (method.kind == Method::NNLS) {
            if (int rc = launch_nnls<T>(ctx, d_mom, n_feat, bias, prm->tol, f32 ? 200 : prm->max_iter, co, gc, fl, d_off + g0)) return rc;
        } else if (int rc = launch_cd<T>(ctx, d_mom, n_feat, bias, method.l1, method.l2, prm->tol, f32 ? 2000 : prm->max_iter,
                                         method.positive, co, nullptr, gc, fl, d_off + g0))
            return rc;
    }
    return PDS_OK;
}

template <typename T>
static int grouped_impl(pds_ctx* ctx, const T* const* cols, int n_feat, int64_t n_rows, const int64_t* offsets,
                        int64_t n_groups, pds_space space, const pds_lr_params* prm, T* coeffs, uint8_t* is_null,
                        bool nullable = false, const uint8_t* const* validity = nullptr, const int64_t* bit_offsets = nullptr,
                        int policy = PDS_NULL_RAISE, T fill_value = T(0),
                        T* pred = nullptr, T* resid = nullptr, uint8_t* row_null = nullptr) {
    const bool want_pred = pred || resid || row_null;
    g_grouped_route = 0;
    if (!ctx || !cols || !offsets || !prm || (!coeffs && !want_pred)) return fail(PDS_ERR_INVALID, "null argument");
    if (want_pred && nullable) return fail(PDS_ERR_UNSUPPORTED, "grouped pred: null-free frames only");
    if (n_feat < 1) return fail(PDS_ERR_INVALID, "need at least one feature column");
    if (n_groups <= 0 || n_rows <= 0) return fail(PDS_ERR_EMPTY, "Empty data");
    const Method method = pick_method(prm);
    PDS_HIP_CHECK(hipSetDevice(ctx->device));
    const int bias = prm->add_bias ? 1 : 0, pp = n_feat + bias, q = n_feat + 2;
    const bool big = n_feat > kMaxFeatWide;
    static const int64_t chunk_env = [] { const char* e = dev_env("PDS_GROUPED_CHUNK_MB"); return e ? std::max<int64_t>(1, std::atoll(e)) : 0; }();
    const int64_t chunk_mb = chunk_env ? chunk_env : ((n_feat > 16 && n_feat <= kMaxFeatWide) ? 2048 : 128);
    int64_t chunk = std::max<int64_t>(big ? 64 : 4096, (int64_t)(chunk_mb << 20) / (int64_t)(sizeof(T) * q * q));
    chunk = std::min(chunk, n_groups);
    size_t need = 131072 + sizeof(T) * (size_t)chunk * q * q;
    need += (size_t)n_groups * 4 + (size_t)chunk * (pp * sizeof(T) + 1) + 4096;
    if (n_feat > 16 && n_feat <= 64) need += solve_wave_workspace(n_feat, bias, chunk, sizeof(T)) + 512;
    if (n_feat > 16 && n_feat <= 32) need += grouped_mid_fused_workspace(ctx->num_cus, n_feat, bias) + 512;
    if (big) need += (size_t)n_groups * (n_feat + 1) * sizeof(T*) + moments_wide_workspace(ctx->num_cus, n_feat, n_rows) + 8192;
    if (space == PDS_HOST || !coeffs) need += (size_t)(n_groups + 1) * 8 + (size_t)n_groups * (pp * sizeof(T) + 1) + 4096;
    T *d_pred = nullptr, *d_resid = nullptr;
    uint8_t* d_rn = nullptr;
    StagedOuts row_outs(space == PDS_HOST, (size_t)n_rows);
    row_outs.add(&d_pred, pred, 1);
    row_outs.add(&d_resid, resid, 1);
    row_outs.add(&d_rn, row_null, 1);
    need += row_outs.bytes();
    if (nullable) {
        if (policy < PDS_NULL_RAISE || policy > PDS_NULL_IGNORE) return fail(PDS_ERR_INVALID, "Invalid NullPolicy.");
        need += (1 << 20) + null_policy_workspace(n_feat + 1, n_rows, sizeof(T)) + (size_t)(n_groups + 1) * 8 + 4096;
        if (space == PDS_HOST) need += (size_t)(n_feat + 1) * ((size_t)n_rows / 8 + 4096);
    }
    if (int rc = ws_reserve(ctx, need)) return rc;
    DeviceCols<T> dc;
    if (int rc = make_device_cols<T>(ctx, cols, (const T*)nullptr, n_feat, n_rows, space, dc)) return rc;
    const int64_t* d_off = offsets;
    T* d_coeffs = coeffs;
    uint8_t* d_null = is_null;
    const size_t co_bytes = ((size_t)n_groups * pp * sizeof(T) + 255) & ~(size_t)255;
    const bool small_out = space == PDS_HOST && coeffs && !want_pred &&
                           co_bytes + (size_t)n_groups + (size_t)(n_groups + 1) * 8 <= ((size_t)48 << 10);
    if (space == PDS_DEVICE && !coeffs) {
        char* blk = reinterpret_cast<char*>(ws_take(ctx, co_bytes + (size_t)n_groups));
        d_coeffs = reinterpret_cast<T*>(blk);
        if (!d_null) d_null = reinterpret_cast<uint8_t*>(blk + co_bytes);
    }
    if (space == PDS_HOST) {
        int64_t* t = reinterpret_cast<int64_t*>(ws_take(ctx, (size_t)(n_groups + 1) * 8));
        if (small_out) {
            if (int rc = ensure_pinned(ctx, (size_t)128 << 10)) return rc;
            char* pin_off = static_cast<char*>(ctx->pinned) + ((size_t)64 << 10);
            std::memcpy(pin_off, offsets, (size_t)(n_groups + 1) * 8);
            PDS_HIP_CHECK(hipMemcpyAsync(t, pin_off, (size_t)(n_groups + 1) * 8, hipMemcpyHostToDevice, ctx->stream));
        } else {
            PDS_HIP_CHECK(hipMemcpyAsync(t, offsets, (size_t)(n_groups + 1) * 8, hipMemcpyHostToDevice, ctx->stream));
        }
        d_off = t;
        char* blk = reinterpret_cast<char*>(ws_take(ctx, co_bytes + (size_t)n_groups));
        d_coeffs = reinterpret_cast<T*>(blk);
        d_null = reinterpret_cast<uint8_t*>(blk + co_bytes);
    } else if (!d_null) {
        d_null = reinterpret_cast<uint8_t*>(ws_take(ctx, (size_t)n_groups));
    }
    if (nullable) {
        const int nc = n_feat + 1;
        std::vector<const T*> ref_order(nc);
        ref_order[0] = dc.h_ptrs[n_feat];
        for (int c = 0; c < n_feat; ++c) ref_order[c + 1] = dc.h_ptrs[c];
        std::vector<const uint8_t*> bms(nc, nullptr);
        std::vector<int64_t> boff(nc, 0);
        for (int c = 0; c < nc; ++c) {
            boff[c] = bit_offsets ? bit_offsets[c] : 0;
            const uint8_t* b = validity ? validity[c] : nullptr;
            if (b && space == PDS_HOST) {
                const size_t bytes = (size_t)((boff[c] + n_rows + 7) / 8);
                uint8_t* d = reinterpret_cast<uint8_t*>(ws_take(ctx, bytes));
                PDS_HIP_CHECK(hipMemcpyAsync(d, b, bytes, hipMemcpyHostToDevice, ctx->stream));
                b = d;
            }
            bms[c] = b;
        }
        NullPrepared<T> prep;
        if (int rc = apply_null_policy<T>(ctx, ref_order, bms, boff, n_rows, policy, fill_value, prep)) return rc;
        if (prep.dropped) {
            int64_t* off2 = reinterpret_cast<int64_t*>(ws_take(ctx, (size_t)(n_groups + 1) * 8));
            if (int rc = remap_group_offsets(ctx, d_off, n_groups, prep.d_rank, n_rows, prep.n_kept, off2)) return rc;
            d_off = off2;
        }
        DeviceCols<T> dk;
        dk.nc = nc;
        dk.h_ptrs.resize(nc);
        for (int c = 0; c < n_feat; ++c) dk.h_ptrs[c] = prep.cols[c + 1];
        dk.h_ptrs[n_feat] = prep.cols[0];
        dk.h_ptrs.resize(std::max(nc, 18), dk.h_ptrs[0]);
        dk.d_ptrs = reinterpret_cast<const T**>(ws_take(ctx, sizeof(T*) * dk.h_ptrs.size()));
        PDS_HIP_CHECK(hipMemcpyAsync(dk.d_ptrs, dk.h_ptrs.data(), sizeof(T*) * dk.h_ptrs.size(), hipMemcpyHostToDevice, ctx->stream));
        PDS_HIP_CHECK(hipStreamSynchronize(ctx->stream));
        dc = dk;
        n_rows = prep.n_kept;
        if (n_rows == 0) return fail(PDS_ERR_EMPTY, "Empty data");
    }
    T* d_mom = reinterpret_cast<T*>(ws_take(ctx, sizeof(T) * (size_t)chunk * q * q));
    SolveParams sp{n_feat, bias, prm->solver, prm->l2_reg, prm->singular_x_tol, 0};
    {
        const char* piv0 = dev_env("PDS_GROUPED_PIVOTED");
        if (piv0 && piv0[0] == '1' && sp.solver == PDS_SOLVER_CHOLESKEY) sp.solver = PDS_SOLVER_QR;
    }
    const char* unfused_env = dev_env("PDS_GROUPED_UNFUSED");
    const char* piv_env = dev_env("PDS_GROUPED_PIVOTED");
    const bool want_piv = !(sp.gate_tol > 0.0) || (piv_env && piv_env[0] == '1');
    if (big) {
        if (int rc = grouped_big<T>(ctx, dc, n_feat, d_off, n_groups, chunk, method, prm, sp, d_mom, d_coeffs, d_null)) return rc;
    } else if (method.kind != Method::OLS) {
        const bool f32 = sizeof(T) == 4;
        for (int64_t g0 = 0; g0 < n_groups; g0 += chunk) {
            const int64_t gc = std::min(chunk, n_groups - g0);
            if (int rc = launch_grouped_moments<T>(ctx, dc, n_feat, d_off + g0, gc, d_mom)) return rc;
            if (method.kind == Method::NNLS) {
                if (int rc = launch_nnls<T>(ctx, d_mom, n_feat, bias, prm->tol, f32 ? 200 : prm->max_iter, d_coeffs + g0 * pp, gc,
                                            d_null + g0, d_off + g0))
                    return rc;
            } else if (int rc = launch_cd<T>(ctx, d_mom, n_feat, bias, method.l1, method.l2, prm->tol,
                                             f32 ? 2000 : prm->max_iter, method.positive, d_coeffs + g0 * pp, nullptr, gc,
                                             d_null + g0, d_off + g0))
                return rc;
        }
    } else if (n_feat <= 16 && !want_piv && !(unfused_env && unfused_env[0] == '1') && n_groups < (1ll << 31)) {
        if (int rc = launch_grouped_fused<T>(ctx, dc, n_feat, n_rows, d_off, n_groups, sp, d_coeffs, d_null, d_mom, chunk)) return rc;
    } else {
        bool mid_done = false;
        {
            const char* mf = dev_env("PDS_GROUPED_MID_FUSED");
            if (n_feat > 16 && n_feat <= 32 && !want_piv && !(mf && mf[0] == '0')) {
                void* d_fws = ws_take(ctx, grouped_mid_fused_workspace(ctx->num_cus, n_feat, bias));
                const int rcf = launch_grouped_mid_fused<T>(ctx, dc, n_feat, n_rows, d_off, n_groups, sp, d_coeffs, d_null, d_fws);
                if (rcf == PDS_OK) mid_done = true;
                else if (rcf != PDS_ERR_UNSUPPORTED) return rcf;
                g_grouped_route = mid_done ? 1 : 2;
            }
        }
        void* d_wave_ws = (!mid_done && n_feat > 16 && n_feat <= 64 && !want_piv) ? ws_take(ctx, solve_wave_workspace(n_feat, bias, chunk, sizeof(T))) : nullptr;
        for (int64_t g0 = 0; g0 < n_groups && !mid_done; g0 += chunk) {
            const int64_t gc = std::min(chunk, n_groups - g0);
            bool streamed = false;
            if constexpr (std::is_same<T, double>::value) {
                static const bool stream_off = [] { const char* e = dev_env("PDS_GROUPED_STREAM"); return e && e[0] == '0'; }();
                if (n_feat >= 28 && n_feat <= 64 && !stream_off) {
                    if (int rc = launch_grouped_moments_stream(ctx, dc, n_feat, n_rows, d_off + g0, gc, d_mom)) return rc;
                    streamed = true;
                }
            }
            if (!streamed)
                if (int rc = launch_grouped_moments<T>(ctx, dc, n_feat, d_off + g0, gc, d_mom)) return rc;
            int rcw = want_piv ? PDS_ERR_UNSUPPORTED
                               : launch_solve_wave<T>(ctx, d_mom, gc, sp, d_coeffs + g0 * pp, d_null + g0, d_off + g0, d_wave_ws);
            if (rcw == PDS_ERR_UNSUPPORTED) rcw = launch_solve<T>(ctx, d_mom, gc, sp, d_coeffs + g0 * pp, d_null + g0, nullptr, d_off + g0);
            if (rcw) return rcw;
        }
    }
    if (want_pred) {
        row_outs.place([&](size_t b) { return ws_take(ctx, b); });
        if (int rc = launch_grouped_pred<T>(ctx, dc.d_ptrs, n_feat, bias, n_rows, d_off, n_groups, d_coeffs, d_null, nullptr, d_pred,
                                            d_resid, d_rn))
            return rc;
        if (int rc = staged_copy_back(ctx, row_outs, (size_t)n_rows)) return rc;
    }
    if (small_out) {
        char* pin = static_cast<char*>(ctx->pinned);
        PDS_HIP_CHECK(hipMemcpyAsync(pin, d_coeffs, co_bytes + (size_t)n_groups, hipMemcpyDeviceToHost, ctx->stream));
        PDS_HIP_CHECK(hipStreamSynchronize(ctx->stream));
        std::memcpy(coeffs, pin, (size_t)n_groups * pp * sizeof(T));
        if (is_null) std::memcpy(is_null, pin + co_bytes, (size_t)n_groups);
        return PDS_OK;
    }
    if (space == PDS_HOST) {
        if (coeffs) PDS_HIP_CHECK(hipMemcpyAsync(coeffs, d_coeffs, (size_t)n_groups * pp * sizeof(T), hipMemcpyDeviceToHost, ctx->stream));
        if (is_null) PDS_HIP_CHECK(hipMemcpyAsync(is_null, d_null, (size_t)n_groups, hipMemcpyDeviceToHost, ctx->stream));
    }
    PDS_HIP_CHECK(hipStreamSynchronize(ctx->stream));
    return PDS_OK;
}

template <typename T>
static int grouped_weighted_impl(pds_ctx* ctx, const T* const* cols, const T* weights, int n_feat, int64_t n_rows,
                                 const int64_t* offsets, int64_t n_groups, pds_space space, const pds_lr_params* prm, T* coeffs,
                                 uint8_t* is_null,
                                 T* pred = nullptr, T* resid = nullptr, uint8_t* row_null = nullptr, const uint32_t* d_perm = nullptr) {
    const bool want_pred = pred || resid || row_null;
    if (!ctx || !cols || !weights || !offsets || !prm || (!coeffs && !want_pred)) return fail(PDS_ERR_INVALID, "null argument");
    if (n_feat < 1) return fail(PDS_ERR_INVALID, "need at least one feature column");
    if (n_groups <= 0 || n_rows <= 0) return fail(PDS_ERR_EMPTY, "Empty data");
    PDS_HIP_CHECK(hipSetDevice(ctx->device));
    const int bias = prm->add_bias ? 1 : 0, pf = n_feat + bias, nc_in = n_feat + 1;
    const auto up = Bump::up;
    const size_t col_bytes = up((size_t)n_rows * sizeof(T));
    T *d_co = nullptr, *d_pred = nullptr, *d_resid = nullptr;
    uint8_t *d_nu = nullptr, *d_rn = nullptr;
    StagedOuts outs(space == PDS_HOST, (size_t)n_groups), row_outs(space == PDS_HOST, (size_t)n_rows);
    outs.add(&d_co, coeffs, pf, StagedOuts::kScratch);
    outs.add(&d_nu, is_null, 1, StagedOuts::kScratch);
    if (want_pred) {
        row_outs.add(&d_pred, pred, 1, StagedOuts::kOutRoom);
        row_outs.add(&d_resid, resid, 1, StagedOuts::kOutRoom);
        row_outs.add(&d_rn, row_null, 1, StagedOuts::kOutRoom);
    }
    size_t need = col_bytes * (pf + 1) + up(sizeof(T*) * (size_t)std::max(nc_in, 18)) + outs.bytes() + row_outs.bytes() + 4096;
    if (space == PDS_HOST) need += col_bytes * (nc_in + 1) + up((size_t)(n_groups + 1) * 8);
    if (int rc = ensure_ws(ctx, ctx->wkeyed, need)) return rc;
    Bump w{static_cast<char*>(ctx->wkeyed.ptr)};
    std::vector<const T*> src = frame_cols<T>(cols, n_feat, weights);
    const int64_t* d_off = offsets;
    if (space == PDS_HOST) {
        if (int rc = cols_to_device<T>(ctx, w, src, n_rows)) return rc;
        int64_t* doff = w.take<int64_t>((size_t)n_groups + 1);
        PDS_HIP_CHECK(hipMemcpyAsync(doff, offsets, (size_t)(n_groups + 1) * 8, hipMemcpyHostToDevice, ctx->stream));
        d_off = doff;
    }
    const T* d_w = src[nc_in];
    outs.place(w);
    std::vector<const T*> scaled(pf + 1);
    for (int c = 0; c < nc_in; ++c) {
        T* d = w.take<T>((size_t)n_rows);
        if (int rc = launch_scale_sqrt_w<T>(ctx, src[c], d_w, n_rows, d)) return rc;
        scaled[c] = d;
    }
    if (bias) {
        T* d = w.take<T>((size_t)n_rows);
        if (int rc = launch_scale_sqrt_w<T>(ctx, (const T*)nullptr, d_w, n_rows, d)) return rc;
        scaled[nc_in] = d;
    }
    pds_lr_params p2 = *prm;
    p2.add_bias = 0;
    p2.l1_reg = 0.0;
    p2.l2_reg = 0.0;
    p2.positive = 0;
    p2.singular_x_tol = 0.0;
    if (int rc = grouped_impl<T>(ctx, scaled.data(), pf, n_rows, d_off, n_groups, PDS_DEVICE, &p2, d_co, d_nu)) return rc;
    if (want_pred) {
        src.pop_back();
        std::vector<const T*> tbl;
        const T** d_tbl = nullptr;
        if (int rc = kernel_order_table<T>(ctx, w, src, n_feat, tbl, d_tbl)) return rc;
        row_outs.place(w);
        if (int rc = launch_grouped_pred<T>(ctx, d_tbl, n_feat, bias, n_rows, d_off, n_groups, d_co, d_nu, d_perm, d_pred, d_resid, d_rn))
            return rc;
        if (int rc = staged_copy_back(ctx, row_outs, (size_t)n_rows)) return rc;
        PDS_HIP_CHECK(hipStreamSynchronize(ctx->stream));
    }
    if (space == PDS_HOST) {
        if (int rc = staged_copy_back(ctx, outs, (size_t)n_groups)) return rc;
        PDS_HIP_CHECK(hipStreamSynchronize(ctx->stream));
    }
    return PDS_OK;
}

template <typename T>
static int solve_partition_table(pds_ctx* ctx, const KeyedPartitionState& st, int n_feat, int64_t n_groups, const int64_t* d_offsets,
                                 const pds_lr_params* prm, T* d_coeffs, uint8_t* d_null) {
    const Method method = pick_method(prm);
    const int bias = prm->add_bias ? 1 : 0, pp = n_feat + bias, q = n_feat + 2;
    int64_t chunk = std::max<int64_t>(4096, (int64_t)(128ll << 20) / (int64_t)(sizeof(T) * q * q));
    chunk = std::min(chunk, n_groups);
    if (int rc = ws_reserve(ctx, 131072 + sizeof(T) * (size_t)chunk * q * q)) return rc;
    T* d_mom = reinterpret_cast<T*>(ws_take(ctx, sizeof(T) * (size_t)chunk * q * q));
    SolveParams sp{n_feat, bias, prm->solver == PDS_SOLVER_SVD ? PDS_SOLVER_QR : prm->solver, prm->l2_reg, prm->singular_x_tol, 0};
    const bool f32 = sizeof(T) == 4;
    if (method.kind == Method::OLS && pp <= 16 && (sp.solver != PDS_SOLVER_CHOLESKEY || sp.gate_tol > 0.0)) {
        static const bool expand = [] { const char* e = dev_env("PDS_PART_EXPAND"); return e && e[0] == '1'; }();
        if (!expand) {
            TriSource tri;
            tri.table = st.table;
            tri.ids = st.ids;
            tri.nvp = st.nvp;
            tri.pc = st.pc;
            return launch_solve_reg<T>(ctx, nullptr, n_groups, sp, d_coeffs, d_null, d_offsets, &tri);
        }
    }
    for (int64_t g0 = 0; g0 < n_groups; g0 += chunk) {
        const int64_t gc = std::min(chunk, n_groups - g0);
        if (int rc = keyed_partition_records<T>(ctx, st, n_feat, g0, gc, d_mom)) return rc;
        KernelTimer timer(ctx, kKindSolve);
        if (method.kind == Method::OLS) {
            if (int rc = launch_solve<T>(ctx, d_mom, gc, sp, d_coeffs + g0 * pp, d_null + g0, nullptr, d_offsets + g0)) return rc;
        } else if (method.kind == Method::NNLS) {
            if (int rc = launch_nnls<T>(ctx, d_mom, n_feat, bias, prm->tol, f32 ? 200 : prm->max_iter, d_coeffs + g0 * pp, gc, d_null + g0,
                                        d_offsets + g0))
                return rc;
        } else if (int rc = launch_cd<T>(ctx, d_mom, n_feat, bias, method.l1, method.l2, prm->tol, f32 ? 2000 : prm->max_iter, method.positive,
                                         d_coeffs + g0 * pp, nullptr, gc, d_null + g0, d_offsets + g0)) {
            return rc;
        }
    }
    return PDS_OK;
}

template <typename T>
struct ByKeyPlace {
    virtual int at(int64_t n_groups, int64_t** out_keys, T** coeffs, uint8_t** is_null) = 0;
    virtual void unsorted() = 0;
    virtual ~ByKeyPlace() = default;
};

template <typename T>
static int lr_by_key_impl(pds_ctx* ctx, const T* const* cols, const int64_t* keys, int n_feat, int64_t n_rows, pds_space space,
                          const pds_lr_params* prm, int64_t max_groups, int64_t* out_keys, T* coeffs, uint8_t* is_null,
                          int64_t* n_groups,
                          const T* weights = nullptr, T* pred = nullptr, T* resid = nullptr, uint8_t* row_null = nullptr,
                          ByKeyPlace<T>* place = nullptr) {
    const bool want_pred = pred || resid || row_null;
    const bool want_coef = out_keys || coeffs || place;
    g_by_key_route = -1;
    g_by_key_info[0] = g_by_key_info[1] = g_by_key_info[2] = g_by_key_info[3] = 0;
    if (!ctx || !cols || !keys || !prm) return fail(PDS_ERR_INVALID, "null argument");
    if (!want_pred && !place && (!out_keys || !coeffs || !n_groups)) return fail(PDS_ERR_INVALID, "null argument");
    if (place && space != PDS_HOST) return fail(PDS_ERR_INVALID, "sliced fits take host frames");
    if (want_coef && !place && (!out_keys || !coeffs)) return fail(PDS_ERR_INVALID, "out_keys and coeffs come together");
    if (n_feat < 1) return fail(PDS_ERR_INVALID, "need at least one feature column");
    if (n_rows <= 0) return fail(PDS_ERR_EMPTY, "Empty data");
    if (!want_coef) max_groups = n_rows;
    if (max_groups < 1) return fail(PDS_ERR_INVALID, "max_groups must be positive");
    PDS_HIP_CHECK(hipSetDevice(ctx->device));
    const int nc = n_feat + 1 + (weights ? 1 : 0), pp = n_feat + (prm->add_bias ? 1 : 0);
    const size_t col_bytes = Bump::up((size_t)n_rows * sizeof(T));
    const bool host = space == PDS_HOST;
    StageTrace tr(ctx, "pds_lr_by_key");
    const bool force_sort = ctx->opt_keyed_sort || (prm->solver == PDS_SOLVER_SVD && prm->singular_x_tol > 0.0);
    const bool part_candidate = !force_sort && !weights && n_feat <= 16 && !place;
    const int part_shift = part_candidate ? keyed_partition_shift<T>(n_feat) : -1;
    KeyOrder ko;
    if (int rc = keyed_order_check(ctx, keys, n_rows, space, true, part_shift, ko)) return rc;
// ... 129 lines not shown
```

polars_ds_extension_amd/csrc/common.hpp:

```cpp
#pragma once
#include <hip/hip_runtime.h>
#include <cmath>
#include <cstdint>
#include <cstdio>
#include <cstring>
#include <string>
#include <type_traits>
#include <vector>

#include "../../include/pds_lstsq.h"

#define PDS_WAVE_LDS_SYNC()                                   \
    do {                                                      \
        asm volatile("s_waitcnt lgkmcnt(0)" ::: "memory");   \
        __builtin_amdgcn_wave_barrier();                      \
    } while (0)

#ifndef PDS_RCP_NEWTON
#define PDS_RCP_NEWTON 2
#endif

namespace pds {

#if defined(__HIPCC__)
template <typename T>
using gptr = const __attribute__((address_space(1))) T*;
template <typename T>
__device__ __forceinline__ gptr<T> as_global(const T* p) {
    return (gptr<T>)p;
}
#endif


template <int LO, int HI, typename F>
inline bool dispatch_width(int n, F&& f) {
    if constexpr (LO > HI) {
        return false;
    } else {
        if (n != LO) return dispatch_width<LO + 1, HI>(n, f);
        f(std::integral_constant<int, LO>{});
        return true;
    }
}

void set_error(const std::string& msg);
int fail(int code, const std::string& msg);

#define PDS_HIP_CHECK(expr)                                                                     \
    do {                                                                                        \
        hipError_t _e = (expr);                                                                 \
        if (_e != hipSuccess)                                                                   \
            return pds::fail(PDS_ERR_HIP, std::string(#expr) + ": " + hipGetErrorString(_e));  \
    } while (0)

constexpr int kMaxFeatSmall = 16;
constexpr int kMaxFeatWide = 64;
constexpr int kTileBytesPerLane = 16;

constexpr int kPartD = 0, kPartXY = 256, kPartCS = 272, kPartYY = 288, kPartYS = 289, kPartSW = 290;
constexpr int kPartY1 = 291, kPartY2 = 292;
constexpr int kPartStride = 296;

struct Workspace {
    void* ptr = nullptr;
    size_t bytes = 0;
};

}

struct pds_ctx {
    int device = 0;
    hipStream_t stream = nullptr;
    bool own_stream = false;
    int num_cus = 256;
    double* partials = nullptr;
    pds::Workspace ws;
    size_t ws_used = 0;
    std::vector<void*> ws_spill;
    long long ws_spill_count = 0;
    pds::Workspace stage;
    pds::Workspace solve_ws;
    pds::Workspace keyed;
    pds::Workspace wkeyed;
    unsigned* mark_count = nullptr;
    unsigned* mark_host = nullptr;
    unsigned* mark_host_dev = nullptr;
    int* wait_timeouts = nullptr;
    bool mark_dirty = false;
    void* pinned = nullptr;
    size_t pinned_bytes = 0;
    void* pinned_in = nullptr;
    size_t pinned_in_bytes = 0;
    bool timing = false;
    std::vector<hipEvent_t> ev_pool;
    struct EvPair { int kind; hipEvent_t a, b; };
    std::vector<EvPair> ev_pending;
    bool opt_keyed_sort = false;
    bool opt_wide_f32_native = false;
    int64_t opt_glm_split_rows = 0;
    int64_t opt_report_chunk_groups = 0;
    int64_t opt_mixed_split_rows = 0;
    int64_t opt_cluster_split_rows = 0;
    int64_t opt_cluster_waves = 0;
    int64_t opt_fused_waves = 0;
    int64_t opt_fused_late_permille = 0;
    double kind_ms[9] = {0, 0, 0, 0, 0, 0, 0, 0, 0};
    long long kind_count[9] = {0, 0, 0, 0, 0, 0, 0, 0, 0};
    std::vector<float> kind_samples[9];
    int64_t opt_multi_route = 0;
    int64_t opt_multi_waves = 0;
    int64_t opt_within_split_rows = 0;
    int64_t opt_within2_accel = 0;
    int64_t opt_rolling_waves = 0;
};

namespace pds {

#ifdef PDS_DEV_SWITCHES
inline const char* dev_env(const char* name) { return std::getenv(name); }
#else
inline const char* dev_env(const char*) { return nullptr; }
#endif

enum { kKindMoments = 0, kKindGroupedMoments = 1, kKindSolve = 2, kKindPass2 = 3, kKindRolling = 4, kKindIter = 5, kKindSweep1 = 6, kKindSweep2 = 7, kKindGraph = 8,
       kNumKinds = 9 };
struct KernelTimer {
    pds_ctx* ctx;
    int kind;
    hipEvent_t a = nullptr, b = nullptr;
    KernelTimer(pds_ctx* c, int k);
    ~KernelTimer();
};

int ensure_ws(pds_ctx* ctx, Workspace& w, size_t bytes);
int ensure_pinned(pds_ctx* ctx, size_t bytes);
int ws_reserve(pds_ctx* ctx, size_t total_bytes);
void* ws_take(pds_ctx* ctx, size_t bytes);

template <typename T>
struct DeviceCols {
    const T** d_ptrs = nullptr;
    std::vector<const T*> h_ptrs;
    int nc = 0;
};

template <typename T>
int make_device_cols(pds_ctx* ctx, const T* const* cols , const T* weights, int n_feat,
                     int64_t n_rows, pds_space space, DeviceCols<T>& out);

struct IrlsArgs {
    int link = 0, variance = 0, init = 0;
    double y_mean = 0.0;
    const void* inv = nullptr;
    int hc_pow = 0;
    int y_sums = 0;
};

template <typename T>
int launch_moments(pds_ctx* ctx, const DeviceCols<T>& dc, int n_feat, int64_t n_rows, bool weighted,
                   T* d_moments ,
                   const T* d_beta_resid = nullptr, int bias_resid = 0, double* d_sums_resid = nullptr,
                   double* d_moments_f64 = nullptr,
                   const IrlsArgs* irls = nullptr,
                   double* d_ysums = nullptr);
template <typename T>
int launch_irls_working_wide(pds_ctx* ctx, const DeviceCols<T>& dc, int n_feat, int64_t n_rows, int bias, const T* d_beta,
                             const IrlsArgs& ia, T* d_w, T* d_z);
template <typename T>
int launch_moments_rowmajor(pds_ctx* ctx, const T* d_X, int64_t ld, const T* d_y, int n_feat, int64_t n_rows, T* d_moments,
                            double* d_moments_f64 = nullptr);
template <typename T>
int launch_sum_moment_slots(pds_ctx* ctx, const double* d_slots, int nslots, int len, T* d_out);

template <typename T>
int launch_moments_wide(pds_ctx* ctx, const DeviceCols<T>& dc, int n_feat, int64_t n_rows, bool weighted, T* d_moments);
size_t moments_wide_workspace(int num_cus, int n_feat, int64_t n_rows, bool weighted = false);
size_t moments_mid_workspace(int num_cus);
template <typename T>
int launch_moments_mid(pds_ctx* ctx, const DeviceCols<T>& dc, int n_feat, int64_t n_rows, bool weighted, T* d_moments);

template <typename T>
int launch_grouped_moments(pds_ctx* ctx, const DeviceCols<T>& dc, int n_feat, const int64_t* d_offsets,
                           int64_t n_groups, T* d_moments, const int32_t* d_group_index = nullptr, bool weighted = false);

struct SolveParams;
template <typename T>
int launch_grouped_fused(pds_ctx* ctx, const DeviceCols<T>& dc, int n_feat, int64_t n_rows, const int64_t* d_offsets,
                         int64_t n_groups, const SolveParams& sp, T* d_coeffs, uint8_t* d_flags, T* d_mom_scratch,
                         int64_t scratch_groups);

struct SolveParams {
    int p;
    int add_bias;
    int solver;
    double lambda;
    double gate_tol;
    int lambda_on_bias;
};
template <typename T>
int launch_solve(pds_ctx* ctx, const T* d_moments, int64_t n_sys, const SolveParams& sp, T* d_coeffs,
                 uint8_t* d_flags, T* d_inv_out, const int64_t* d_rows_per_sys );

template <typename T>
int launch_solve_marked(pds_ctx* ctx, const T* d_rec, int64_t n_sys, const SolveParams& sp, T* d_coeffs, uint8_t* d_flags,
                        const int64_t* d_rows_per_sys);

template <typename T>
int launch_solve_big(pds_ctx* ctx, const T* d_moments, int64_t n_sys, const SolveParams& sp, T* d_coeffs, uint8_t* d_flags,
                     T* d_inv_out);

struct TriSource {
    const double* table = nullptr;
    const unsigned* ids = nullptr;
    int nvp = 0, pc = 0;
};
template <typename T>
int launch_solve_reg(pds_ctx* ctx, const T* d_moments, int64_t n_sys, const SolveParams& sp, T* d_coeffs,
                     uint8_t* d_flags, const int64_t* d_rows_per_sys, const TriSource* tri = nullptr);

template <typename T>
int launch_solve_wave(pds_ctx* ctx, const T* d_moments, int64_t n_sys, const SolveParams& sp, T* d_coeffs, uint8_t* d_flags,
                      const int64_t* d_rows_per_sys, void* d_ws);
size_t solve_wave_workspace(int n_feat, int add_bias, int64_t n_sys, size_t elem);

template <typename T>
int launch_cd(pds_ctx* ctx, const T* d_moments, int p, int add_bias, double l1, double l2, double tol,
              int max_iter, int positive, T* d_coeffs, int* d_info ,
              int64_t n_sys = 1, uint8_t* d_flags = nullptr, const int64_t* d_rows_per_sys = nullptr,
              double pen_rows = 0.0 ,
              int warm_start = 0 );
template <typename T>
int launch_nnls(pds_ctx* ctx, const T* d_moments, int p, int add_bias, double tol, int max_iter, T* d_coeffs,
                int64_t n_sys = 1, uint8_t* d_flags = nullptr, const int64_t* d_rows_per_sys = nullptr);

template <typename T>
int launch_grouped_pred(pds_ctx* ctx, const T* const* d_cols, int n_feat, int bias, int64_t n_rows, const int64_t* d_off,
                        int64_t n_groups, const T* d_coeffs, const uint8_t* d_flags, const uint32_t* d_perm, T* d_pred, T* d_resid,
                        uint8_t* d_row_null);

template <typename T>
int launch_grouped_pred_by_id(pds_ctx* ctx, const T* const* d_cols, int n_feat, int bias, int64_t n_rows, const int64_t* d_keys,
                              const int64_t* d_kmin, const uint32_t* d_rank, int64_t n_groups, const T* d_coeffs, const uint8_t* d_flags,
                              T* d_pred, T* d_resid, uint8_t* d_row_null);
template <typename T>
inline int grouped_pred_table_stride(int pp) {
    const int b = pp * (int)sizeof(T);
    return b <= 64 ? 64 / (int)sizeof(T) : (b <= 128 ? 128 / (int)sizeof(T) : pp);
}
template <typename T>
int launch_grouped_pred_by_id_table(pds_ctx* ctx, const T* const* d_cols, int n_feat, int bias, int64_t n_rows, const int64_t* d_keys,
                                    const int64_t* d_kmin, const uint32_t* d_ids , int64_t n_groups, const T* d_coeffs,
                                    const uint8_t* d_flags, T* d_table , T* d_pred, T* d_resid, uint8_t* d_row_null);
template <typename T>
int launch_grouped_irls(pds_ctx* ctx, const T* const* d_cols, int n_feat, int bias, int64_t n_rows, const int64_t* d_off,
                        int64_t n_groups, int link, int variance, double tol, int max_iter, int64_t split_rows, T* d_coeffs,
                        int32_t* d_n_iter, uint8_t* d_null, T* d_pred , uint8_t* d_row_null ,
                        const uint32_t* d_perm ,
                        int64_t* d_long_list, unsigned* d_long_count, int64_t long_cap, double l1_reg = 0.0, double l2_reg = 0.0);
template <typename T>
int launch_grouped_irls_wo(pds_ctx* ctx, const T* const* d_cols, int n_feat, int bias, int64_t n_rows, const int64_t* d_off,
                           int64_t n_groups, int link, int variance, double tol, int max_iter, int64_t split_rows, T* d_coeffs,
                           int32_t* d_n_iter, uint8_t* d_null, T* d_pred , uint8_t* d_row_null ,
                           const uint32_t* d_perm , int64_t* d_long_list, unsigned* d_long_count, int64_t long_cap);
template <typename T>
int launch_glm_wo_sums(pds_ctx* ctx, const T* d_y, const T* d_pw, int64_t n_rows, double* d_out4);
template <typename T>
int launch_irls_working_wo(pds_ctx* ctx, const DeviceCols<T>& dc, int n_feat, int64_t n_rows, int bias, const T* d_beta, const IrlsArgs& ia,
                           const T* d_pw, const T* d_off, T* d_w, T* d_z);
constexpr double kGiCdInner = 0.1;
constexpr int kGiCdSweeps = 1000;
template <typename T>
int launch_glm_pred_range(pds_ctx* ctx, const T* const* d_cols, int n_feat, int bias, int64_t r0, int64_t r1, const T* d_beta,
                          const uint8_t* d_null_flag, int link, T* d_pred, uint8_t* d_row_null, const uint32_t* d_perm,
                          const T* d_offset = nullptr );
template <typename T>
struct GlmReportDev {
    T *se, *z, *p, *lo, *hi, *cov, *deviance, *null_deviance, *pearson, *dispersion;
    int64_t* df_resid;
    uint8_t* report_null;
};
constexpr int kGlmReportRec = 280;
template <typename T>
int launch_grouped_glm_report(pds_ctx* ctx, const T* const* d_cols, int n_feat, int bias, int64_t n_rows, const int64_t* d_off,
                              int64_t n_groups, int link, int variance, int64_t split_rows, const T* d_coeffs, const uint8_t* d_null,
                              const GlmReportDev<T>& out, int64_t* d_long_list, unsigned* d_long_count, int64_t long_cap);
template <typename T>
int launch_grouped_glm_report_pieces(pds_ctx* ctx, const T* const* d_cols, int n_feat, int bias, const int64_t* d_off, int link,
                                     int variance, const T* d_coeffs, const GlmReportDev<T>& out, const int64_t* d_pieces,
                                     int64_t n_pieces, const int64_t* d_fin, int64_t n_fin, double* d_rec);
template <typename T>
int launch_grouped_glm_report_wo(pds_ctx* ctx, const T* const* d_cols, int n_feat, int bias, int64_t n_rows, const int64_t* d_off,
                                 int64_t n_groups, int link, int variance, int64_t split_rows, const T* d_coeffs, const uint8_t* d_null,
                                 const GlmReportDev<T>& out, int64_t* d_long_list, unsigned* d_long_count, int64_t long_cap);
template <typename T>
int launch_grouped_glm_report_wo_pieces(pds_ctx* ctx, const T* const* d_cols, int n_feat, int bias, const int64_t* d_off, int link,
                                        int variance, const T* d_coeffs, const GlmReportDev<T>& out, const int64_t* d_pieces,
                                        int64_t n_pieces, const int64_t* d_fin, int64_t n_fin, double* d_rec);
template <typename T>
int launch_grouped_rcond(pds_ctx* ctx, const T* const* d_cols, int n_feat, int bias, int64_t n_rows, const int64_t* d_off,
                         int64_t n_groups, double l2_reg, double rcond, T* d_coeffs, T* d_svals, uint8_t* d_null);
template <typename T>
int launch_grouped_multi(pds_ctx* ctx, const T* const* d_cols, int n_feat, int n_targets, int bias, int64_t n_rows, const int64_t* d_off,
                         int64_t n_groups, double l2_reg, double gate_tol, bool mark_suspects, T* d_coeffs, uint8_t* d_flags,
                         int32_t* d_mark_list, unsigned* d_mark_count);
template <typename T>
int launch_multi_scatter(pds_ctx* ctx, const T* d_co, const uint8_t* d_fl, const int32_t* d_list, int64_t n, int t, int k, int pp, bool first,
                         T* d_coeffs, uint8_t* d_flags);
template <typename T>
int launch_multi_null_fill(pds_ctx* ctx, uint8_t* d_flags, const int32_t* d_list, int64_t n, int kpp, bool check_finite, T* d_coeffs);
template <typename T>
int launch_multi_extract(pds_ctx* ctx, const T* d_coeffs, int64_t n_groups, int t, int k, int pp, T* d_out);
int launch_multi_offsets_check(pds_ctx* ctx, const int64_t* d_off, int64_t n_groups, int64_t n_rows, unsigned* d_bad);
constexpr int kMixedRecW = 0, kMixedRecXY = 256, kMixedRecCM = 272, kMixedRecYY = 288, kMixedRecC = 289, kMixedRecCY = 290, kMixedRecLD = 291;
constexpr int kMixedRecStride = 296;
int launch_sum_records(pds_ctx* ctx, const double* d_rec, int n_rec, double* d_stage, double* d_out, bool compensated);
struct MixedChunks {
    int64_t n_chunks = 0, n_long = 0;
    const int64_t *d_chunk_r0 = nullptr, *d_chunk_n = nullptr, *d_chunk_g = nullptr, *d_chunk_first = nullptr;
    const int64_t *d_long_g = nullptr, *d_long_c0 = nullptr, *d_long_nc = nullptr, *d_long_first = nullptr, *d_long_n = nullptr;
    double* d_sums = nullptr;
    unsigned* d_varies = nullptr;
};
int mixed_stats_blocks(const pds_ctx* ctx, int64_t n_work);
int mixed_profile_blocks(const pds_ctx* ctx, int64_t n_groups);
template <typename T>
int launch_mixed_stats(pds_ctx* ctx, const T* const* d_cols, int n_feat, const int64_t* d_off, int64_t n_groups, int64_t split_rows,
                       const MixedChunks& ch, const double* d_beta0, double* d_means, unsigned* d_flags, double* d_partials,
                       double* d_stage, double* d_w);
int launch_mixed_profile(pds_ctx* ctx, const double* d_means, int n_feat, const int64_t* d_off, int64_t n_groups, double gamma,
                         double* d_partials, double* d_stage, double* d_out);
constexpr int kClusterScoreStride = 18;
struct ClusterChunks {
    int64_t n_chunks = 0, n_long = 0;
    const int64_t *d_chunk_r0 = nullptr, *d_chunk_n = nullptr;
    const int64_t *d_long_c0 = nullptr, *d_long_nc = nullptr;
    double* d_scores = nullptr;
};
int cluster_meat_blocks(const pds_ctx* ctx, int64_t n_work);
template <typename T>
int launch_cluster_meat(pds_ctx* ctx, const T* const* d_cols, int n_feat, const int64_t* d_off, int64_t n_clusters, int64_t split_rows,
                        const ClusterChunks& ch, const T* d_beta, int bias, double* d_partials, double* d_stage, double* d_rec);
int glm_meat_records(const pds_ctx* ctx, int64_t n_rows, int64_t n_clusters, const ClusterChunks& ch);
// ... 194 lines not shown
```

polars_ds_extension_amd/csrc/grouped_fused.hip:

```cpp
#include <type_traits>

#include "grouped_split_dev.hpp"
#include "moments_dev.hpp"
#include "solve_reg_dev.hpp"

namespace pds {

#ifdef PDS_PROFILE_PHASES
__device__ unsigned long long g_phase_cycles[8];
#define PDS_T0() const unsigned long long _t0 = __builtin_amdgcn_s_memtime()
#define PDS_T1(k) prof[k] += __builtin_amdgcn_s_memtime() - _t0
#else
#define PDS_T0() do {} while (0)
#define PDS_T1(k) do {} while (0)
#endif
#if defined(PDS_PROFILE_PHASES) || defined(PDS_PROFILE_TAIL)
#define PDS_WAVE_STAMPS 1
constexpr int kStampWaves = 4096;
__device__ unsigned long long g_wave_stamps[4 * kStampWaves];
static int g_stamp_grid = 0;
#define PDS_STAMP_BEGIN()                                                             \
    const unsigned long long _st_rt = __builtin_amdgcn_s_memrealtime();               \
    const unsigned long long _st_mt = __builtin_amdgcn_s_memtime()
#define PDS_STAMP_END()                                                                                                     \
    do {                                                                                                                    \
        if ((threadIdx.x & 63) == 0 && blockIdx.x < (unsigned)kStampWaves) {                                                \
            unsigned long long* _s = g_wave_stamps + 4 * (size_t)blockIdx.x;                                                \
            _s[0] = _st_rt;                                                                                                 \
            _s[1] = __builtin_amdgcn_s_memrealtime();                                                                       \
            _s[2] = __builtin_amdgcn_s_memtime() - _st_mt;                                                                  \
            _s[3] = (1ull << 63) | ((unsigned long long)__builtin_amdgcn_s_getreg(4 | (31 << 11)) << 8)      \
                    | (unsigned long long)(__builtin_amdgcn_s_getreg(20 | (3 << 11)) & 0xFu);               \
        }                                                                                                                   \
    } while (0)
#define PDS_STAMP_SKIP()                                                                                  \
    do {                                                                                                  \
        if ((threadIdx.x & 63) == 0 && blockIdx.x < (unsigned)kStampWaves) g_wave_stamps[4 * (size_t)blockIdx.x + 3] = 0ull; \
    } while (0)
#else
#define PDS_STAMP_BEGIN() do {} while (0)
#define PDS_STAMP_END() do {} while (0)
#define PDS_STAMP_SKIP() do {} while (0)
#endif

constexpr int kFQ = 18;
constexpr int kFM = kFQ * kFQ;
constexpr int kFTile = 17 * kColStride;
constexpr int kFWaveLds = kFTile + kFM * 8;

template <typename T, bool BIAS>
__device__ __forceinline__ void consume_range(const char* wl, int lane, int rel0, int rel1, WaveAcc& a) {
    const int f = lane & 15, q = lane >> 4;
    const T* xcol = reinterpret_cast<const T*>(wl + f * kColStride) + q;
    const T* ycol = reinterpret_cast<const T*>(wl + kSlotY * kColStride) + q;
    int s0 = rel0 >> 2;
    const int s1 = (rel1 + 3) >> 2;
    using Acc = typename Tile<T>::acc;
    Acc acc;
    double xy, cs, yy, ys;
    if constexpr (sizeof(T) == 8) {
        acc = Acc{a.d[0], a.d[1], a.d[2], a.d[3]};
        xy = a.xy; cs = a.cs; yy = a.yy; ys = a.ys;
    } else {
        acc = Acc{0, 0, 0, 0};
        xy = cs = yy = ys = 0.0;
    }
    T fxy = 0, fcs = 0, fyy = 0, fys = 0;
    auto step_v = [&](T x, T yv) __attribute__((always_inline)) {
        acc = Tile<T>::mfma(x, x, acc);
        if constexpr (sizeof(T) == 8) {
            xy = fma(x, yv, xy);
            if constexpr (BIAS) {
                cs += x;
                ys += yv;
            }
        } else {
            fxy = fmaf(x, yv, fxy);
            if constexpr (BIAS) {
                fcs += x;
                fys += yv;
            }
        }
    };
    auto step = [&](int s, bool masked, int lo, int hi) __attribute__((always_inline)) {
        T x = xcol[4 * s];
        T yv = ycol[4 * s];
        if (masked) {
            const bool in = q >= lo && q < hi;
            x = in ? x : T(0);
            yv = in ? yv : T(0);
        }
        acc = Tile<T>::mfma(x, x, acc);
        if constexpr (sizeof(T) == 8) {
            xy = fma(x, yv, xy);
            if constexpr (BIAS) {
                cs += x;
                ys += yv;
            }
        } else {
            fxy = fmaf(x, yv, fxy);
            if constexpr (BIAS) {
                fcs += x;
                fys += yv;
            }
        }
    };
    if (rel0 & 3) {
        const int lo = rel0 & 3;
        const int hi = min(rel1 - 4 * s0, 4);
        step(s0, true, lo, hi);
        ++s0;
    }
    const int sfull = rel1 >> 2;
    int s = s0;
    for (; s + 4 <= sfull; s += 4) {
        const T x0 = xcol[4 * s], x1 = xcol[4 * s + 4], x2 = xcol[4 * s + 8], x3 = xcol[4 * s + 12];
        const T y0 = ycol[4 * s], y1 = ycol[4 * s + 4], y2 = ycol[4 * s + 8], y3 = ycol[4 * s + 12];
        step_v(x0, y0);
        step_v(x1, y1);
        step_v(x2, y2);
        step_v(x3, y3);
    }
    for (; s < sfull; ++s) step_v(xcol[4 * s], ycol[4 * s]);
    if ((rel1 & 3) && sfull >= s0 && sfull < s1) step(sfull, true, 0, rel1 & 3);
    if constexpr (sizeof(T) == 8) {
        a.d[0] = acc[0]; a.d[1] = acc[1]; a.d[2] = acc[2]; a.d[3] = acc[3];
        a.xy = xy; a.cs = cs; a.yy = yy; a.ys = ys;
    } else {
        a.d[0] += (double)acc[0]; a.d[1] += (double)acc[1]; a.d[2] += (double)acc[2]; a.d[3] += (double)acc[3];
        a.xy += (double)fxy; a.cs += (double)fcs; a.yy += (double)fyy; a.ys += (double)fys;
    }
}

template <typename T, bool BIAS>
__device__ __forceinline__ void consume_range_pack(const char* wl, int lane, int rel0, int rel1, WaveAcc& a) {
    const int f = lane & 15, q = lane >> 4;
    const int roff = q + 4 * (f >> 3);
    const T* xcol = reinterpret_cast<const T*>(wl + (f & 7) * kColStride) + roff;
    const T* ycol = reinterpret_cast<const T*>(wl + kSlotY * kColStride) + roff;
    int s0 = rel0 >> 3;
    const int s1 = (rel1 + 7) >> 3;
    using Acc = typename Tile<T>::acc;
    Acc acc;
    double xy, cs, yy, ys;
    if constexpr (sizeof(T) == 8) {
        acc = Acc{a.d[0], a.d[1], a.d[2], a.d[3]};
        xy = a.xy; cs = a.cs; yy = a.yy; ys = a.ys;
    } else {
        acc = Acc{0, 0, 0, 0};
        xy = cs = yy = ys = 0.0;
    }
    T fxy = 0, fcs = 0, fyy = 0, fys = 0;
    auto step_v = [&](T x, T yv) __attribute__((always_inline)) {
        acc = Tile<T>::mfma(x, x, acc);
        if constexpr (sizeof(T) == 8) {
            xy = fma(x, yv, xy);
            if constexpr (BIAS) {
                cs += x;
                ys += yv;
            }
        } else {
            fxy = fmaf(x, yv, fxy);
            if constexpr (BIAS) {
                fcs += x;
                fys += yv;
            }
        }
    };
    auto step_m = [&](int s) __attribute__((always_inline)) {
        const int r = 8 * s + roff;
        const bool in = r >= rel0 && r < rel1;
        const T x = in ? xcol[8 * s] : T(0);
        const T yv = in ? ycol[8 * s] : T(0);
        step_v(x, yv);
    };
    if (rel0 & 7) {
        step_m(s0);
        ++s0;
    }
    const int sfull = rel1 >> 3;
    int s = s0;
    for (; s + 4 <= sfull; s += 4) {
        const T x0 = xcol[8 * s], x1 = xcol[8 * s + 8], x2 = xcol[8 * s + 16], x3 = xcol[8 * s + 24];
        const T y0 = ycol[8 * s], y1 = ycol[8 * s + 8], y2 = ycol[8 * s + 16], y3 = ycol[8 * s + 24];
        step_v(x0, y0);
        step_v(x1, y1);
        step_v(x2, y2);
        step_v(x3, y3);
    }
    for (; s < sfull; ++s) step_v(xcol[8 * s], ycol[8 * s]);
    if ((rel1 & 7) && sfull >= s0 && sfull < s1) step_m(sfull);
    if constexpr (sizeof(T) == 8) {
        a.d[0] = acc[0]; a.d[1] = acc[1]; a.d[2] = acc[2]; a.d[3] = acc[3];
// ... 99 lines not shown
        }
        if (live && j == 0 && flags) flags[sys] = suspect ? 2 : (is_null ? 1 : 0);
        if constexpr (CHOL) {
            const bool mk = suspect && live && j == 0;
            const unsigned long long mm = __ballot(mk);
            if (mm != 0ull && mark_list) {
                const int leader = __ffsll((long long)mm) - 1;
                unsigned slot = 0;
                if (lane == leader) {
                    slot = atomicAdd(mark_count, (unsigned)__popcll(mm));
                    __hip_atomic_store(mark_host_flag, 1u, __ATOMIC_RELAXED, __HIP_MEMORY_SCOPE_SYSTEM);
                }
                slot = __shfl(slot, leader);
                if (mk) mark_list[slot + __popcll(mm & ((1ull << lane) - 1ull))] = (int32_t)sys;
            }
        }
        PDS_T1(3);
        gbase += npend;
        npend = 0;
    };

    WaveAcc acc;
    zero_acc(acc);
    int64_t g = gl;
    int64_t gs = rlo;
    int64_t ge = offsets[g + 1];
    uint32_t g_left = (uint32_t)(gh - gl);
    int64_t ge_next = offsets[g_left >= 2 ? g + 2 : gh];
    int64_t pos = rlo;

    auto flush_group = [&]() __attribute__((always_inline)) {
        PDS_T0();
        const uint64_t ng = (uint64_t)(ge - gs);
        const bool too_few = (uint32_t)(ng >> 32) == 0u && (uint32_t)ng < (uint32_t)pout;
        {
            const int jj = lane & 15;
            constexpr bool RFOLD = PACK && sizeof(T) == 8;
            auto shl8 = [](double v) __attribute__((always_inline)) {
                int lo = __double2loint(v), hi = __double2hiint(v);
                lo = __builtin_amdgcn_update_dpp(0, lo, 0x108 , 0xf, 0xf, true);
                hi = __builtin_amdgcn_update_dpp(0, hi, 0x108, 0xf, 0xf, true);
                return __hiloint2double(hi, lo);
            };
            if constexpr (RFOLD) {
                const double d0 = acc.d[0] + shl8(acc.d[2]), d1 = acc.d[1] + shl8(acc.d[3]);
                if (jj < 8) {
                    Msc[Tile<T>::drow(lane, 0) + kFQ * jj] = d0;
                    Msc[Tile<T>::drow(lane, 1) + kFQ * jj] = d1;
                }
            } else {
#pragma unroll
                for (int r = 0; r < 4; ++r) Msc[Tile<T>::drow(lane, r) + kFQ * jj] = acc.d[r];
            }
            double xy = xor_sum_q(acc.xy);
            if constexpr (RFOLD) xy += shl8(xy);
            if (lane < (RFOLD ? 8 : 16)) Msc[lane + kFQ * 17] = xy;
            if constexpr (BIAS) {
                double cs = xor_sum_q(acc.cs), ys = xor_sum_q(acc.ys);
                if constexpr (RFOLD) {
                    cs += shl8(cs);
                    ys += shl8(ys);
                }
                if (lane < (RFOLD ? 8 : 16)) Msc[lane + kFQ * 16] = cs;
                if (lane == 0) {
                    Msc[16 + kFQ * 16] = (double)ng;
                    Msc[16 + kFQ * 17] = ys;
                }
                if (PACK && !RFOLD && lane == 8) Msc[17 + kFQ * 17] = ys;
            }
        }
        if constexpr (PACK && sizeof(T) != 8) {
            PDS_WAVE_LDS_SYNC();
            const int fi = lane & 7, fj = lane >> 3;
            const double dsum = Msc[fi + kFQ * fj] + Msc[fi + 8 + kFQ * (fj + 8)];
            double xys = 0.0, css = 0.0, yss = 0.0;
            if (lane < 8) {
                xys = Msc[lane + kFQ * 17] + Msc[lane + 8 + kFQ * 17];
                if constexpr (BIAS) css = Msc[lane + kFQ * 16] + Msc[lane + 8 + kFQ * 16];
            }
            if (BIAS && lane == 0) yss = Msc[16 + kFQ * 17] + Msc[17 + kFQ * 17];
            PDS_WAVE_LDS_SYNC();
            Msc[fi + kFQ * fj] = dsum;
            if (lane < 8) {
                Msc[lane + kFQ * 17] = xys;
                if constexpr (BIAS) Msc[lane + kFQ * 16] = css;
            }
            if (BIAS && lane == 0) Msc[16 + kFQ * 17] = yss;
        }
        if (sp.lambda > 0.0) {
            PDS_WAVE_LDS_SYNC();
            if (lane < p) Msc[lane * (kFQ + 1)] += sp.lambda;
        }
        PDS_WAVE_LDS_SYNC();
        {
            int j = j_in;
            asm volatile("" : "+v"(j));
            const int lj = (j < p) ? j : ZSLOT;
            if (sub == npend) {
                const double* colp = Msc + kFQ * lj;
                if (p >= LPS) {
#pragma unroll
                    for (int i = 0; i < LPS; ++i) {
                        a_p[i] = colp[i];
                        if constexpr (!CHOL) b_p[i] = Msc[i + kFQ * 17];
                    }
                } else {
#pragma unroll
                    for (int i = 0; i < LPS; ++i) {
                        const int li = (i < p) ? i : ZSLOT;
                        a_p[i] = colp[li];
                        if constexpr (!CHOL) b_p[i] = Msc[li + kFQ * 17];
                    }
                }
                if constexpr (CHOL) a_p[LPS] = Msc[lj + kFQ * 17];
                dj_p = (j < pp) ? colp[lj] : 1.0;
                null_p = too_few;
                if constexpr (BIAS) {
                    static_assert(CHOL, "the centred bias form exists for the Cholesky kernel");
                    const double csj = Msc[lj + kFQ * 16];
                    const double nn = (double)ng, sy = Msc[16 + kFQ * 17];
                    const double m = csj / nn;
#pragma unroll
                    for (int i = 0; i < LPS; ++i) {
                        const int li = (p >= LPS || i < p) ? i : ZSLOT;
                        a_p[i] = fma(-Msc[li + kFQ * 16], m, a_p[i]);
                    }
                    a_p[LPS] = fma(-sy, m, a_p[LPS]);
                    cs_p = csj;
                    ys_p = sy;
                    n_p = nn;
                }
            }
        }
        PDS_WAVE_LDS_SYNC();
        zero_acc(acc);
        ++npend;
        PDS_T1(2);
        if (npend == SPW) solve_pending();
    };

    TileRegs<T> regs;
    const int64_t t_first = rlo / TR, t_last = (rhi > rlo) ? (rhi - 1) / TR : t_first - 1;
    auto load_tile = [&](int64_t t) __attribute__((always_inline)) {
        ColPtrs<T> cp;
#pragma unroll
        for (int c = 0; c < 16; ++c) cp.x[c] = as_global(cols[c]);
        cp.y = as_global(cols[p]);
        cp.w = cp.y;
        const int64_t row = t * TR + lane * RPL;
        if ((t + 1) * TR <= n_rows) load_full_tile<T, false>(cp, p, row, regs);
        else load_tail_tile<T, false>(cp, p, row, n_rows, regs);
    };
    if (t_first <= t_last) load_tile(t_first);
    for (int64_t t = t_first;; ++t) {
        const bool have_tile = t <= t_last;
        if (have_tile) {
            {
                PDS_T0();
                store_tile_lds<T, false>(wl, p, lane, regs);
#ifdef PDS_PROFILE_PHASES
                PDS_WAVE_LDS_SYNC();
#endif
                PDS_T1(0);
            }
            PDS_T0();
            if (t + 1 <= t_last) load_tile(t + 1);
            PDS_T1(1);
        }
        const int64_t row0 = t * TR;
        uint32_t rel_end = 0, pos_rel = 0;
        if (have_tile) {
            const uint64_t left = (uint64_t)(rhi - row0);
            rel_end = ((uint32_t)(left >> 32) != 0u || (uint32_t)left > (uint32_t)TR) ? (uint32_t)TR : (uint32_t)left;
            pos_rel = (uint32_t)(pos - row0);
        }
        auto rel_of = [&](int64_t r) __attribute__((always_inline)) {
            const uint64_t d = (uint64_t)(r - (have_tile ? row0 : pos));
            return ((uint32_t)(d >> 32) != 0u) ? 0xFFFFFFFFu : (uint32_t)d;
        };
        uint32_t ge_rel = rel_of(ge);
        while (g_left != 0u && (pos_rel < rel_end || ge_rel <= pos_rel)) {
            if (ge_rel <= pos_rel) {
                flush_group();
                ++g;
                --g_left;
                gs = ge;
                ge = ge_next;
                ge_next = offsets[g_left >= 2u ? g + 2 : gh];
                ge_rel = rel_of(ge);
                continue;
            }
            const uint32_t seg_end = (ge_rel < rel_end) ? ge_rel : rel_end;
            PDS_T0();
            if constexpr (PACK) consume_range_pack<T, BIAS>(wl, lane, (int)pos_rel, (int)seg_end, acc);
            else consume_range<T, BIAS>(wl, lane, (int)pos_rel, (int)seg_end, acc);
            PDS_T1(4);
            pos_rel = seg_end;
        }
        if (have_tile) pos = row0 + pos_rel;
        if (t >= t_last) break;
        PDS_WAVE_LDS_SYNC();
    }
    if (npend > 0) solve_pending();
#ifdef PDS_PROFILE_PHASES
    prof[7] = __builtin_amdgcn_s_memtime() - t_begin;
    if (lane == 0)
        for (int k = 0; k < 8; ++k) atomicAdd(&g_phase_cycles[k], prof[k]);
#endif
    PDS_STAMP_END();
}

template <typename T, int LPS>
static int launch_stream_lps(pds_ctx* ctx, const DeviceCols<T>& dc, int n_feat, const int64_t* d_offsets,
                             int64_t n_groups, int64_t n_rows, const SolveRegDev& sd, bool chol, T* d_coeffs,
                             uint8_t* d_flags, int32_t* d_mark_list, unsigned* d_mark_count, unsigned* d_mark_host) {
    const size_t lds = (size_t)kFWaveLds;
    const int per_cu = std::max(1, (int)((160 * 1024) / lds));
    const int64_t slots = (int64_t)ctx->num_cus * per_cu;
    int64_t nb = std::min<int64_t>(std::max<int64_t>(n_groups / (64 / LPS), 1), slots);
    if (ctx->opt_fused_waves > 0) nb = std::min<int64_t>(nb, ctx->opt_fused_waves);
    const int late_pm = fused_late_permille(nb, slots, ctx->opt_fused_late_permille);
    KernelTimer timer(ctx, kKindGroupedMoments);
    if (!chol) return fail(PDS_ERR_INVALID, "internal: fused grouped kernel is Cholesky-only");
    auto go = [&](auto bias_c, auto pc_c) {
        hipLaunchKernelGGL((grouped_stream_kernel<T, LPS, true, decltype(bias_c)::value, decltype(pc_c)::value>), dim3((unsigned)nb),
                           dim3(64), lds, ctx->stream, dc.d_ptrs, n_feat, d_offsets, n_groups, n_rows, sd, d_coeffs, d_flags, d_mark_list,
                           d_mark_count, d_mark_host, late_pm);
    };
    auto by_pc = [&](auto bias_c) {
        using std::integral_constant;
        constexpr int LO = LPS == 4 ? 1 : LPS / 2 + 1;
        if (n_feat == LPS) return go(bias_c, integral_constant<int, LPS>{});
        if constexpr (sizeof(T) == 8) {
            if (n_feat == LO) return go(bias_c, integral_constant<int, LO>{});
            if constexpr (LPS >= 4) {
                if (n_feat == LO + 1 && LO + 1 < LPS) return go(bias_c, integral_constant<int, (LO + 1 < LPS ? LO + 1 : LPS)>{});
                if (n_feat == LO + 2 && LO + 2 < LPS) return go(bias_c, integral_constant<int, (LO + 2 < LPS ? LO + 2 : LPS)>{});
            }
            if constexpr (LPS == 16) {
                if (n_feat == 12) return go(bias_c, integral_constant<int, 12>{});
                if (n_feat == 13) return go(bias_c, integral_constant<int, 13>{});
                if (n_feat == 14) return go(bias_c, integral_constant<int, 14>{});
                if (n_feat == 15) return go(bias_c, integral_constant<int, 15>{});
            }
        }
        return go(bias_c, integral_constant<int, 0>{});
    };
    if (sd.bias) by_pc(std::true_type{});
    else by_pc(std::false_type{});
    PDS_HIP_CHECK(hipGetLastError());
#ifdef PDS_WAVE_STAMPS
    g_stamp_grid = (int)nb;
#endif
    return PDS_OK;
}

static int ensure_mark_state(pds_ctx* ctx) {
    if (ctx->mark_count) return PDS_OK;
    PDS_HIP_CHECK(hipMalloc(reinterpret_cast<void**>(&ctx->mark_count), 256));
    ctx->mark_dirty = true;
    PDS_HIP_CHECK(hipHostMalloc(reinterpret_cast<void**>(&ctx->mark_host), 64, hipHostMallocMapped | hipHostMallocCoherent));
    *ctx->mark_host = 0u;
    PDS_HIP_CHECK(hipHostGetDevicePointer(reinterpret_cast<void**>(&ctx->mark_host_dev), ctx->mark_host, 0));
    return PDS_OK;
}

template <typename T>
__global__ void scatter_marked_kernel(const T* __restrict__ co_c, const uint8_t* __restrict__ fl_c, const int32_t* __restrict__ list,
                                      int64_t n, int pp, T* __restrict__ coeffs, uint8_t* __restrict__ flags) {
    const int64_t i = (int64_t)blockIdx.x * blockDim.x + threadIdx.x;
    if (i >= n * pp) return;
    const int64_t k = i / pp;
    const int c = (int)(i - k * pp);
    const int64_t g = list[k];
    coeffs[g * pp + c] = co_c[i];
    if (c == 0) flags[g] = fl_c[k] ? 1 : 0;
}

template <typename T>
int launch_grouped_fused(pds_ctx* ctx, const DeviceCols<T>& dc, int n_feat, int64_t n_rows, const int64_t* d_offsets,
                         int64_t n_groups, const SolveParams& sp, T* d_coeffs, uint8_t* d_flags, T* d_mom_scratch,
                         int64_t scratch_groups) {
    SolveRegDev sd;
    sd.p = sp.p;
    sd.bias = sp.add_bias ? 1 : 0;
    sd.pp = sp.p + sd.bias;
    sd.lambda_on_bias = sp.lambda_on_bias;
    sd.lambda = sp.lambda;
    sd.gate_on = sp.gate_tol > 0.0 ? 1 : 0;
    sd.ln_tol = sd.gate_on ? std::log(sp.gate_tol) : 0.0;
    sd.inv_tol = sd.gate_on ? 1.0 / sp.gate_tol : HUGE_VAL;
    if (n_groups <= 0) return PDS_OK;
    if (n_groups >= (1ll << 31)) return fail(PDS_ERR_INVALID, "internal: fused grouped kernel counts groups per wave in 32 bits");
    const char* piv = dev_env("PDS_GROUPED_PIVOTED");
    const bool chol = sd.gate_on && !(piv && piv[0] == '1');
    const bool second_pass = chol && sp.solver != PDS_SOLVER_CHOLESKEY && d_flags && d_mom_scratch && scratch_groups > 0;
    sd.sus_tol = second_pass ? std::sqrt(sd.inv_tol) : 0.0;
    int32_t* d_list = nullptr;
    unsigned* d_count = nullptr;
    unsigned* d_host = nullptr;
    if (second_pass) {
        if (int rc0 = ensure_mark_state(ctx)) return rc0;
        d_list = reinterpret_cast<int32_t*>(ws_take(ctx, (size_t)n_groups * sizeof(int32_t)));
        if (!d_list) return fail(PDS_ERR_HIP, "workspace allocation failed");
        d_count = ctx->mark_count;
        d_host = ctx->mark_host_dev;
        *ctx->mark_host = 0u;
        if (ctx->mark_dirty) PDS_HIP_CHECK(hipMemsetAsync(d_count, 0, sizeof(unsigned), ctx->stream));
        ctx->mark_dirty = true;
    }
    int rc;
    if (sd.p <= 4) rc = launch_stream_lps<T, 4>(ctx, dc, n_feat, d_offsets, n_groups, n_rows, sd, chol, d_coeffs, d_flags, d_list, d_count, d_host);
    else if (sd.p <= 8) rc = launch_stream_lps<T, 8>(ctx, dc, n_feat, d_offsets, n_groups, n_rows, sd, chol, d_coeffs, d_flags, d_list, d_count, d_host);
    else rc = launch_stream_lps<T, 16>(ctx, dc, n_feat, d_offsets, n_groups, n_rows, sd, chol, d_coeffs, d_flags, d_list, d_count, d_host);
    if (rc || !second_pass) return rc;
    PDS_HIP_CHECK(hipStreamSynchronize(ctx->stream));
    if (__atomic_load_n(ctx->mark_host, __ATOMIC_ACQUIRE) == 0u) {
        ctx->mark_dirty = false;
        return PDS_OK;
    }
    unsigned h_count = 0;
    PDS_HIP_CHECK(hipMemcpyAsync(&h_count, d_count, sizeof(unsigned), hipMemcpyDeviceToHost, ctx->stream));
    PDS_HIP_CHECK(hipMemsetAsync(d_count, 0, sizeof(unsigned), ctx->stream));
    PDS_HIP_CHECK(hipStreamSynchronize(ctx->stream));
    ctx->mark_dirty = false;
    const int64_t marked = (int64_t)h_count;
    if (marked == 0) return PDS_OK;
    const int pp = sd.pp;
    const int64_t chunk = std::min<int64_t>(scratch_groups, marked);
    T* co_c = reinterpret_cast<T*>(ws_take(ctx, (size_t)chunk * pp * sizeof(T)));
    uint8_t* fl_c = reinterpret_cast<uint8_t*>(ws_take(ctx, (size_t)chunk));
    if (!co_c || !fl_c) return fail(PDS_ERR_HIP, "workspace allocation failed");
    for (int64_t k0 = 0; k0 < marked; k0 += chunk) {
        const int64_t kc = std::min(chunk, marked - k0);
        if (int rc2 = launch_grouped_moments<T>(ctx, dc, n_feat, d_offsets, kc, d_mom_scratch, d_list + k0)) return rc2;
        if (int rc2 = launch_solve_marked<T>(ctx, d_mom_scratch, kc, sp, co_c, fl_c, nullptr)) return rc2;
        hipLaunchKernelGGL((scatter_marked_kernel<T>), dim3((unsigned)((kc * pp + 255) / 256)), dim3(256), 0, ctx->stream, co_c, fl_c,
                           d_list + k0, kc, pp, d_coeffs, d_flags);
        PDS_HIP_CHECK(hipGetLastError());
    }
    return PDS_OK;
}

#ifdef PDS_PROFILE_PHASES
extern "C" int pds_debug_phase_cycles(unsigned long long* out, int reset) {
    unsigned long long z[8] = {0, 0, 0, 0, 0, 0, 0, 0};
    if (hipMemcpyFromSymbol(out, HIP_SYMBOL(g_phase_cycles), sizeof(z)) != hipSuccess) return -1;
    if (reset && hipMemcpyToSymbol(HIP_SYMBOL(g_phase_cycles), z, sizeof(z)) != hipSuccess) return -1;
    return 0;
}
#endif

#ifdef PDS_WAVE_STAMPS
extern "C" int pds_debug_wave_stamps(unsigned long long* out, int max_waves) {
    const int n = std::min(std::min(g_stamp_grid, kStampWaves), max_waves);
    if (n <= 0) return 0;
    if (hipMemcpyFromSymbol(out, HIP_SYMBOL(g_wave_stamps), (size_t)n * 4 * sizeof(unsigned long long)) != hipSuccess) return -1;
    return n;
}
#endif

template int launch_grouped_fused<double>(pds_ctx*, const DeviceCols<double>&, int, int64_t, const int64_t*, int64_t,
                                          const SolveParams&, double*, uint8_t*, double*, int64_t);
template int launch_grouped_fused<float>(pds_ctx*, const DeviceCols<float>&, int, int64_t, const int64_t*, int64_t,
                                         const SolveParams&, float*, uint8_t*, float*, int64_t);

}
```

polars_ds_extension_amd/lstsq.py:

```python
from __future__ import annotations

import contextlib
import ctypes as C
import threading
from typing import Sequence

import numpy as np

from . import _lib, config

__all__ = [
    "Context", "default_context", "lin_reg", "lin_reg_report", "lin_reg_by", "lin_reg_report_by", "lin_reg_report_by_key", "rolling_lin_reg", "rolling_lin_reg_by", "rolling_lin_reg_by_key", "recursive_lin_reg_by",
    "recursive_lin_reg_by_key", "glm_by", "glm_by_key", "glm_report_by", "glm_report_by_key", "logistic_reg", "mixed_reml", "mixed_reml_profile",
    "recursive_lin_reg", "lin_reg_w_rcond", "lin_reg_w_rcond_by", "lin_reg_w_rcond_by_key", "lin_reg_multi_by", "lin_reg_multi_by_key", "elastic_net_fit", "report_fit_from_moments", "report_partials", "report_finish", "gram_moments", "lin_reg_from_moments", "query_ar_coeffs",
]


def _is_torch(a) -> bool:
    return type(a).__module__.startswith("torch")


def _dtype():
    return np.float64 if config.LIN_REG_EXPR_F64 else np.float32


def _suffix() -> str:
    return "_f64" if config.LIN_REG_EXPR_F64 else "_f32"


class _Cols:

    def __init__(self, y, xs: Sequence, weights=None):
        dt = _dtype()
        arrs = [y, *xs] + ([weights] if weights is not None else [])
        if any(_is_torch(a) for a in arrs):
            import torch

            tdt = torch.float64 if dt == np.float64 else torch.float32
            keep = []
            for a in arrs:
                if not _is_torch(a):
                    a = torch.as_tensor(np.asarray(a))
                if not a.is_cuda:
                    a = a.cuda()
                keep.append(a.to(tdt).contiguous())
            self.space = _lib.PDS_DEVICE
            ptrs = [int(a.data_ptr()) for a in keep]
            self.n_rows = int(keep[0].shape[0])
            self.device_index = keep[0].device.index or 0
            self.torch_device = keep[0].device
        else:
            keep = [np.ascontiguousarray(np.asarray(a), dtype=dt) for a in arrs]
            self.space = _lib.PDS_HOST
            ptrs = [int(a.ctypes.data) for a in keep]
            self.n_rows = int(keep[0].shape[0])
            self.device_index = None
        for a in keep:
            if a.ndim != 1 or int(a.shape[0]) != self.n_rows:
                raise ValueError("all columns must be 1-D and of equal length")
        self.keep = keep
        self.n_feat = len(xs)
        nb = 1 + self.n_feat
        self.cols = (C.c_void_p * nb)(*ptrs[:nb])
        self.weights = C.c_void_p(ptrs[nb]) if weights is not None else C.c_void_p(None)


class Context:

    def __init__(self, device: int = 0, stream=None):
        self._lib = _lib.load()
        self._h = C.c_void_p()
        _lib.check(self._lib.pds_ctx_create(int(device), C.byref(self._h)))
        self.device = int(device)
        if stream is not None:
            self.set_stream(stream)

    def set_stream(self, stream) -> None:
        raw = getattr(stream, "cuda_stream", stream)
        _lib.check(self._lib.pds_ctx_set_stream(self._h, C.c_void_p(int(raw) if raw else None)))
        self._stream_raw = int(raw) if raw else 0

    def follow_torch_stream(self, device) -> None:
        import torch

        raw = int(torch.cuda.current_stream(device).cuda_stream)
        if getattr(self, "_stream_raw", -1) != raw:
            self.set_stream(raw)
            self._stream_raw = raw

    def synchronize(self) -> None:
        _lib.check(self._lib.pds_ctx_synchronize(self._h))

    def set_option(self, name: str, value) -> None:
        _lib.check(self._lib.pds_ctx_set_option(self._h, str(name).encode(), C.c_longlong(int(value))))

    def get_option(self, name: str) -> int:
        v = C.c_longlong(0)
        _lib.check(self._lib.pds_ctx_get_option(self._h, str(name).encode(), C.byref(v)))
        return int(v.value)

    @property
    def num_cus(self) -> int:
        return int(self._lib.pds_ctx_num_cus(self._h))

    def signal_post(self, word_addr: int, value: int) -> None:
        _lib.check(self._lib.pds_signal_post(self._h, C.c_void_p(int(word_addr)), C.c_uint(int(value) & 0xFFFFFFFF)))

    def signal_wait(self, words_addr: int, n_words: int, value: int, timeout_ms: int = 2000) -> None:
        _lib.check(self._lib.pds_signal_wait(self._h, C.c_void_p(int(words_addr)), int(n_words), C.c_uint(int(value) & 0xFFFFFFFF), int(timeout_ms)))

    def signal_wait_timeouts(self) -> int:
        n = C.c_int(0)
        _lib.check(self._lib.pds_signal_wait_status(self._h, C.byref(n)))
        return int(n.value)

    WORKSPACES = ("scratch", "stage", "solve", "keyed", "wkeyed")

    def workspace_bytes(self, which: str = "keyed") -> int:
        return int(self._lib.pds_ctx_workspace_bytes(self._h, self.WORKSPACES.index(which)))

    KINDS = ("moments", "grouped_moments", "solve", "pass2", "rolling", "iterative", "sweep_factor1", "sweep_factor2", "graph")

    def set_timing(self, enable: bool) -> None:
        _lib.check(self._lib.pds_ctx_set_timing(self._h, int(bool(enable))))

    def get_timing(self, reset: bool = True) -> dict:
        nk = len(self.KINDS)
        ms = (C.c_double * nk)()
        cnt = (C.c_longlong * nk)()
        _lib.check(self._lib.pds_ctx_get_timing(self._h, ms, cnt, nk, int(bool(reset))))
        return {k: (ms[i], int(cnt[i])) for i, k in enumerate(self.KINDS)}

    def get_timing_samples(self, kind: str, reset: bool = True) -> list:
        buf = (C.c_double * 4096)()
        n = int(self._lib.pds_ctx_get_timing_samples(self._h, self.KINDS.index(kind), buf, 4096, int(bool(reset))))
        if n < 0:
            raise ValueError(kind)
        return [float(buf[i]) for i in range(n)]

    def close(self) -> None:
        if getattr(self, "_h", None) and self._h.value:
            self._lib.pds_ctx_destroy(self._h)
            self._h = C.c_void_p()

    def __del__(self):
        try:
            self.close()
        except Exception:
            pass

    def fn(self, name: str):
        return getattr(self._lib, name + _suffix())


_tls = threading.local()


def default_context() -> Context:
    ctx = getattr(_tls, "ctx", None)
    if ctx is None:
        ctx = _tls.ctx = Context(0)
    return ctx


def _follow(ctx: "Context", cols: "_Cols") -> None:
    if cols.space == _lib.PDS_DEVICE:
        ctx.follow_torch_stream(cols.torch_device)


def _params(add_bias, l1_reg, l2_reg, tol, solver, positive, max_iter, singular_x_tol) -> _lib.LRParams:
    if singular_x_tol is None:
        singular_x_tol = 1e-12 if config.LIN_REG_EXPR_F64 else 1e-6
    return _lib.LRParams(int(bool(add_bias)), float(l1_reg), float(l2_reg), float(tol), _lib.SOLVERS.get(solver, 0),
                         int(bool(positive)), int(max_iter), float(singular_x_tol))


def _out_like(cols: _Cols, shape):
    if cols.space == _lib.PDS_DEVICE:
        import torch

        tdt = torch.float64 if config.LIN_REG_EXPR_F64 else torch.float32
        t = torch.empty(shape, dtype=tdt, device=cols.keep[0].device)
        return t, C.c_void_p(int(t.data_ptr()))
    a = np.empty(shape, dtype=_dtype())
    return a, C.c_void_p(a.ctypes.data)


def _out_int(cols: _Cols, n, dtype: str):
    if cols.space == _lib.PDS_DEVICE:
        import torch

        t = torch.empty(n, dtype=getattr(torch, dtype), device=cols.keep[0].device)
        return t, C.c_void_p(int(t.data_ptr()))
    a = np.empty(n, dtype=dtype)
    return a, C.c_void_p(a.ctypes.data)


def _out_u8(cols: _Cols, n):
    return _out_int(cols, n, "uint8")


def parse_null_policy(value: str):
    v = str(value).lower()
    if v == "raise":
        return 0, 0.0
    if v == "skip":
        return 1, 0.0
    if v == "zero":
        return 2, 0.0
    if v == "one":
        return 2, 1.0
    if v == "ignore":
        return 3, 0.0
    try:
        return 2, float(value)
    except ValueError:
        raise ValueError("Invalid NullPolicy.") from None


def _is_arrow(a) -> bool:
    return type(a).__module__.startswith("pyarrow")


def _arrow_parts(a, dt):
    import pyarrow as pa

    if isinstance(a, pa.ChunkedArray):
        a = a.combine_chunks() if a.num_chunks != 1 else a.chunk(0)
    want = pa.float64() if dt == np.float64 else pa.float32()
    if a.type != want:
        a = a.cast(want)
    vbuf, dbuf = a.buffers()
    vals = np.frombuffer(dbuf, dtype=dt)[a.offset : a.offset + len(a)]
    has_nulls = vbuf is not None and a.null_count > 0
    return vals, (vbuf.address if has_nulls else 0), a.offset, (a, vbuf, dbuf)


def _lin_reg_arrow(x, target, add_bias, return_pred, null_policy, prm, ctx):
    dt = _dtype()
    parts = [_arrow_parts(c, dt) if _is_arrow(c) else (np.ascontiguousarray(np.asarray(c), dtype=dt), 0, 0, None)
             for c in (target, *x)]
    n = len(parts[0][0])
    if any(len(pt[0]) != n for pt in parts):
        raise ValueError("all columns must be 1-D and of equal length")
    nc = len(parts)
    cols = (C.c_void_p * nc)(*[pt[0].ctypes.data for pt in parts])
    vals = (C.c_void_p * nc)(*[pt[1] or None for pt in parts])
    offs = (C.c_int64 * nc)(*[pt[2] for pt in parts])
    code, fill = parse_null_policy(null_policy)
    pp = nc - 1 + int(bool(add_bias))
    coeffs = np.empty(pp, dtype=dt)
    is_null, n_used = C.c_int(0), C.c_int64(0)
# ... 1730 lines not shown
```

Measured before the change: 414.8 million regressions/s.

## Return grouped lstsq stream-ordered with on-device fixup of marked groups

When the caller supplies its own stream and inputs live on the device, the fused grouped lstsq path now skips the final host synchronize and returns asynchronously. Rank-gated groups that need a second pass are refit by a new device-side fixup kernel, replacing the host round trip that read the mark count. The device column-pointer table is cached per context and rewritten by a tiny kernel only when the pointers change, avoiding a per-call H2D copy. This adds an opt-out option, debug hooks and extra profiling stamps, and risks ordering bugs if the caller reads results without synchronizing.

```diff
diff --git a/polars_ds_extension_amd/_lib.py b/polars_ds_extension_amd/_lib.py
--- a/polars_ds_extension_amd/_lib.py
+++ b/polars_ds_extension_amd/_lib.py
@@ -197,6 +197,9 @@
                                                                                             C.c_int, C.c_int, C.c_int64] + [C.c_void_p] * 3
         if hasattr(lib, "pds_absorb_components_i32"):
             lib.pds_absorb_components_i32.argtypes = [C.c_void_p, C.c_void_p, C.c_int64, C.c_void_p, C.c_int64, C.c_int64, C.c_int] + [C.c_void_p] * 6
+        if hasattr(lib, "pds_debug_mark_state"):
+            lib.pds_debug_mark_state.argtypes = [C.c_void_p, C.POINTER(C.c_uint)]
+            lib.pds_debug_last_return_async.argtypes = [C.c_void_p]
         if hasattr(lib, "pds_ctx_workspace_bytes"):
             lib.pds_ctx_workspace_bytes.argtypes = [C.c_void_p, C.c_int]
             lib.pds_ctx_workspace_bytes.restype = C.c_longlong
diff --git a/polars_ds_extension_amd/csrc/capi.hip b/polars_ds_extension_amd/csrc/capi.hip
--- a/polars_ds_extension_amd/csrc/capi.hip
+++ b/polars_ds_extension_amd/csrc/capi.hip
@@ -109,6 +109,7 @@
     if (ctx->keyed.ptr) (void)hipFree(ctx->keyed.ptr);
     if (ctx->wkeyed.ptr) (void)hipFree(ctx->wkeyed.ptr);
     if (ctx->mark_count) (void)hipFree(ctx->mark_count);
+    if (ctx->col_table_dev) (void)hipFree(ctx->col_table_dev);
     if (ctx->wait_timeouts) (void)hipFree(ctx->wait_timeouts);
     if (ctx->mark_host) (void)hipHostFree(ctx->mark_host);
     if (ctx->pinned) (void)hipHostFree(ctx->pinned);
@@ -129,6 +130,8 @@
     if (ctx->own_stream && ctx->stream) (void)hipStreamDestroy(ctx->stream);
     ctx->stream = reinterpret_cast<hipStream_t>(hip_stream);
     ctx->own_stream = false;
+    ctx->caller_stream = true;
+    ctx->col_table_valid = false;
     return PDS_OK;
 }
 
@@ -163,7 +166,11 @@
         ctx->opt_multi_route = (int64_t)value;
     } else if (n == "grouped_multi_waves") ctx->opt_multi_waves = value > 0 ? (int64_t)value : 0;
     else if (n == "rolling_waves") ctx->opt_rolling_waves = value > 0 ? (int64_t)value : 0;
-    else return fail(PDS_ERR_INVALID, "unknown context option: " + n);
+    else if (n == "blocking_return") {
+        if (value != 0 && value != 1) return fail(PDS_ERR_INVALID, "blocking_return: 0 (stream-ordered where the header allows it) or 1 (always synchronise)");
+        PDS_HIP_CHECK(hipStreamSynchronize(ctx->stream));
+        ctx->opt_blocking_return = (int64_t)value;
+    } else return fail(PDS_ERR_INVALID, "unknown context option: " + n);
     return PDS_OK;
 }
 
@@ -184,6 +191,7 @@
     else if (n == "grouped_multi_route") *value = ctx->opt_multi_route;
     else if (n == "grouped_multi_waves") *value = ctx->opt_multi_waves;
     else if (n == "rolling_waves") *value = ctx->opt_rolling_waves;
+    else if (n == "blocking_return") *value = ctx->opt_blocking_return;
     else return fail(PDS_ERR_INVALID, "unknown context option: " + n);
     return PDS_OK;
 }
@@ -861,12 +869,18 @@
 int pds_lr_grouped_f64(pds_ctx* ctx, const double* const* cols, int n_feat, int64_t n_rows,
                        const int64_t* group_offsets, int64_t n_groups, pds_space space, const pds_lr_params* prm,
                        double* coeffs, uint8_t* is_null) {
-    return grouped_impl<double>(ctx, cols, n_feat, n_rows, group_offsets, n_groups, space, prm, coeffs, is_null);
+    const int rc = grouped_impl<double>(ctx, cols, n_feat, n_rows, group_offsets, n_groups, space, prm, coeffs, is_null, false, nullptr,
+                                        nullptr, PDS_NULL_RAISE, 0.0, nullptr, nullptr, nullptr, true);
+    if (rc && ctx) ctx->col_table_valid = false;
+    return rc;
 }
 int pds_lr_grouped_f32(pds_ctx* ctx, const float* const* cols, int n_feat, int64_t n_rows,
                        const int64_t* group_offsets, int64_t n_groups, pds_space space, const pds_lr_params* prm,
                        float* coeffs, uint8_t* is_null) {
-    return grouped_impl<float>(ctx, cols, n_feat, n_rows, group_offsets, n_groups, space, prm, coeffs, is_null);
+    const int rc = grouped_impl<float>(ctx, cols, n_feat, n_rows, group_offsets, n_groups, space, prm, coeffs, is_null, false, nullptr,
+                                       nullptr, PDS_NULL_RAISE, 0.0f, nullptr, nullptr, nullptr, true);
+    if (rc && ctx) ctx->col_table_valid = false;
+    return rc;
 }
 
 int pds_lr_grouped_nullable_f64(pds_ctx* ctx, const double* const* cols, const uint8_t* const* validity,
@@ -1241,6 +1255,16 @@
 }
 int pds_debug_last_multi_route(void) { return pds::g_multi_route; }
 int pds_debug_last_grouped_route(void) { return pds::g_grouped_route; }
+int pds_debug_last_return_async(const pds_ctx* ctx) { return ctx ? ctx->last_return_async : 0; }
+int pds_debug_mark_state(pds_ctx* ctx, unsigned* out2) {
+    if (!ctx || !out2) return pds::fail(PDS_ERR_INVALID, "null argument");
+    out2[0] = out2[1] = 0u;
+    PDS_HIP_CHECK(hipSetDevice(ctx->device));
+    PDS_HIP_CHECK(hipStreamSynchronize(ctx->stream));
+    if (!ctx->mark_count) return PDS_OK;
+    PDS_HIP_CHECK(hipMemcpy(out2, ctx->mark_count, 2 * sizeof(unsigned), hipMemcpyDeviceToHost));
+    return PDS_OK;
+}
 int pds_debug_last_by_key_route(int* info ) {
     if (info)
         for (int i = 0; i < 4; ++i) info[i] = pds::g_by_key_info[i];
diff --git a/polars_ds_extension_amd/csrc/capi_core.hpp b/polars_ds_extension_amd/csrc/capi_core.hpp
--- a/polars_ds_extension_amd/csrc/capi_core.hpp
+++ b/polars_ds_extension_amd/csrc/capi_core.hpp
@@ -98,9 +98,17 @@
 
 constexpr size_t kSmallFrameBytes = (size_t)1 << 20;
 
+struct ColTable18 {
+    const void* p[18];
+};
+__global__ void write_col_table_kernel(ColTable18 t, const void** __restrict__ dst) {
+    if (threadIdx.x < 18) dst[threadIdx.x] = t.p[threadIdx.x];
+}
+static inline bool ctx_stream_ordered(const pds_ctx* ctx) { return ctx->caller_stream && !ctx->opt_blocking_return && !ctx->timing; }
+
 template <typename T>
 int make_device_cols(pds_ctx* ctx, const T* const* cols, const T* weights, int n_feat, int64_t n_rows,
-                     pds_space space, DeviceCols<T>& out) {
+                     pds_space space, DeviceCols<T>& out, bool table_on_stream) {
     const int nc = n_feat + 1 + (weights ? 1 : 0);
     out.nc = nc;
     out.h_ptrs.resize(nc);
@@ -147,6 +155,20 @@
         }
     }
     out.h_ptrs.resize(std::max(nc, 18), out.h_ptrs[0]);
+    if (table_on_stream && space == PDS_DEVICE && out.h_ptrs.size() == 18) {
+        if (!ctx->col_table_dev) PDS_HIP_CHECK(hipMalloc(reinterpret_cast<void**>(&ctx->col_table_dev), 256));
+        ColTable18 t;
+        for (int c = 0; c < 18; ++c) t.p[c] = out.h_ptrs[c];
+        if (!ctx->col_table_valid || std::memcmp(t.p, ctx->col_table_host, sizeof(t.p)) != 0) {
+            ctx->col_table_valid = false;
+            hipLaunchKernelGGL(write_col_table_kernel, dim3(1), dim3(64), 0, ctx->stream, t, ctx->col_table_dev);
+            PDS_HIP_CHECK(hipGetLastError());
+            std::memcpy(ctx->col_table_host, t.p, sizeof(t.p));
+            ctx->col_table_valid = true;
+        }
+        out.d_ptrs = reinterpret_cast<const T**>(ctx->col_table_dev);
+        return PDS_OK;
+    }
     out.d_ptrs = reinterpret_cast<const T**>(ws_take(ctx, sizeof(T*) * out.h_ptrs.size()));
     PDS_HIP_CHECK(hipMemcpyAsync(out.d_ptrs, out.h_ptrs.data(), sizeof(T*) * out.h_ptrs.size(), hipMemcpyHostToDevice, ctx->stream));
     return PDS_OK;
diff --git a/polars_ds_extension_amd/csrc/capi_grouped.hpp b/polars_ds_extension_amd/csrc/capi_grouped.hpp
--- a/polars_ds_extension_amd/csrc/capi_grouped.hpp
+++ b/polars_ds_extension_amd/csrc/capi_grouped.hpp
@@ -69,8 +69,10 @@
                         int64_t n_groups, pds_space space, const pds_lr_params* prm, T* coeffs, uint8_t* is_null,
                         bool nullable = false, const uint8_t* const* validity = nullptr, const int64_t* bit_offsets = nullptr,
                         int policy = PDS_NULL_RAISE, T fill_value = T(0),
-                        T* pred = nullptr, T* resid = nullptr, uint8_t* row_null = nullptr) {
+                        T* pred = nullptr, T* resid = nullptr, uint8_t* row_null = nullptr,
+                        bool may_stay_on_stream = false) {
     const bool want_pred = pred || resid || row_null;
+    if (ctx) ctx->last_return_async = 0;
     g_grouped_route = 0;
     if (!ctx || !cols || !offsets || !prm || (!coeffs && !want_pred)) return fail(PDS_ERR_INVALID, "null argument");
     if (want_pred && nullable) return fail(PDS_ERR_UNSUPPORTED, "grouped pred: null-free frames only");
@@ -103,8 +105,10 @@
         if (space == PDS_HOST) need += (size_t)(n_feat + 1) * ((size_t)n_rows / 8 + 4096);
     }
     if (int rc = ws_reserve(ctx, need)) return rc;
+    const bool want_stream = may_stay_on_stream && ctx_stream_ordered(ctx) && space == PDS_DEVICE && coeffs && !nullable && !want_pred;
+    bool on_stream = false;
     DeviceCols<T> dc;
-    if (int rc = make_device_cols<T>(ctx, cols, (const T*)nullptr, n_feat, n_rows, space, dc)) return rc;
+    if (int rc = make_device_cols<T>(ctx, cols, (const T*)nullptr, n_feat, n_rows, space, dc, want_stream)) return rc;
     const int64_t* d_off = offsets;
     T* d_coeffs = coeffs;
     uint8_t* d_null = is_null;
@@ -197,7 +201,8 @@
                 return rc;
         }
     } else if (n_feat <= 16 && !want_piv && !(unfused_env && unfused_env[0] == '1') && n_groups < (1ll << 31)) {
-        if (int rc = launch_grouped_fused<T>(ctx, dc, n_feat, n_rows, d_off, n_groups, sp, d_coeffs, d_null, d_mom, chunk)) return rc;
+        on_stream = want_stream;
+        if (int rc = launch_grouped_fused<T>(ctx, dc, n_feat, n_rows, d_off, n_groups, sp, d_coeffs, d_null, d_mom, chunk, &on_stream)) return rc;
     } else {
         bool mid_done = false;
         {
@@ -247,6 +252,11 @@
     if (space == PDS_HOST) {
         if (coeffs) PDS_HIP_CHECK(hipMemcpyAsync(coeffs, d_coeffs, (size_t)n_groups * pp * sizeof(T), hipMemcpyDeviceToHost, ctx->stream));
         if (is_null) PDS_HIP_CHECK(hipMemcpyAsync(is_null, d_null, (size_t)n_groups, hipMemcpyDeviceToHost, ctx->stream));
+    }
+    if (want_stream && on_stream) {
+        ctx->last_return_async = 1;
+        ctx->async_pending = true;
+        return PDS_OK;
     }
     PDS_HIP_CHECK(hipStreamSynchronize(ctx->stream));
     return PDS_OK;
diff --git a/polars_ds_extension_amd/csrc/common.hpp b/polars_ds_extension_amd/csrc/common.hpp
--- a/polars_ds_extension_amd/csrc/common.hpp
+++ b/polars_ds_extension_amd/csrc/common.hpp
@@ -112,6 +112,13 @@
     int64_t opt_within_split_rows = 0;
     int64_t opt_within2_accel = 0;
     int64_t opt_rolling_waves = 0;
+    bool caller_stream = false;
+    int64_t opt_blocking_return = 0;
+    int last_return_async = 0;
+    const void** col_table_dev = nullptr;
+    const void* col_table_host[18] = {};
+    bool col_table_valid = false;
+    bool async_pending = false;
 };
 
 namespace pds {
@@ -146,7 +153,8 @@
 
 template <typename T>
 int make_device_cols(pds_ctx* ctx, const T* const* cols , const T* weights, int n_feat,
-                     int64_t n_rows, pds_space space, DeviceCols<T>& out);
+                     int64_t n_rows, pds_space space, DeviceCols<T>& out,
+                     bool table_on_stream = false);
 
 struct IrlsArgs {
     int link = 0, variance = 0, init = 0;
@@ -187,7 +195,7 @@
 template <typename T>
 int launch_grouped_fused(pds_ctx* ctx, const DeviceCols<T>& dc, int n_feat, int64_t n_rows, const int64_t* d_offsets,
                          int64_t n_groups, const SolveParams& sp, T* d_coeffs, uint8_t* d_flags, T* d_mom_scratch,
-                         int64_t scratch_groups);
+                         int64_t scratch_groups, bool* stay_on_stream = nullptr);
 
 struct SolveParams {
     int p;
diff --git a/polars_ds_extension_amd/csrc/grouped_fused.hip b/polars_ds_extension_amd/csrc/grouped_fused.hip
--- a/polars_ds_extension_amd/csrc/grouped_fused.hip
+++ b/polars_ds_extension_amd/csrc/grouped_fused.hip
@@ -17,15 +17,23 @@
 #if defined(PDS_PROFILE_PHASES) || defined(PDS_PROFILE_TAIL)
 #define PDS_WAVE_STAMPS 1
 constexpr int kStampWaves = 4096;
-__device__ unsigned long long g_wave_stamps[4 * kStampWaves];
+constexpr int kStampWords = 5;
+__device__ unsigned long long g_wave_stamps[kStampWords * kStampWaves];
 static int g_stamp_grid = 0;
 #define PDS_STAMP_BEGIN()                                                             \
     const unsigned long long _st_rt = __builtin_amdgcn_s_memrealtime();               \
+    unsigned long long _st_fl = _st_rt;                                               \
     const unsigned long long _st_mt = __builtin_amdgcn_s_memtime()
+#define PDS_STAMP_FIRST_LOAD()                        \
+    do {                                              \
+        asm volatile("" ::: "memory");                \
+        _st_fl = __builtin_amdgcn_s_memrealtime();    \
+    } while (0)
 #define PDS_STAMP_END()                                                                                                     \
     do {                                                                                                                    \
         if ((threadIdx.x & 63) == 0 && blockIdx.x < (unsigned)kStampWaves) {                                                \
-            unsigned long long* _s = g_wave_stamps + 4 * (size_t)blockIdx.x;                                                \
+            unsigned long long* _s = g_wave_stamps + kStampWords * (size_t)blockIdx.x;                                      \
+            _s[4] = _st_fl;                                                                                                 \
             _s[0] = _st_rt;                                                                                                 \
             _s[1] = __builtin_amdgcn_s_memrealtime();                                                                       \
             _s[2] = __builtin_amdgcn_s_memtime() - _st_mt;                                                                  \
@@ -35,10 +43,11 @@
     } while (0)
 #define PDS_STAMP_SKIP()                                                                                  \
     do {                                                                                                  \
-        if ((threadIdx.x & 63) == 0 && blockIdx.x < (unsigned)kStampWaves) g_wave_stamps[4 * (size_t)blockIdx.x + 3] = 0ull; \
+        if ((threadIdx.x & 63) == 0 && blockIdx.x < (unsigned)kStampWaves) g_wave_stamps[kStampWords * (size_t)blockIdx.x + 3] = 0ull; \
     } while (0)
 #else
 #define PDS_STAMP_BEGIN() do {} while (0)
+#define PDS_STAMP_FIRST_LOAD() do {} while (0)
 #define PDS_STAMP_END() do {} while (0)
 #define PDS_STAMP_SKIP() do {} while (0)
 #endif
@@ -444,6 +453,7 @@
         else load_tail_tile<T, false>(cp, p, row, n_rows, regs);
     };
     if (t_first <= t_last) load_tile(t_first);
+    PDS_STAMP_FIRST_LOAD();
     for (int64_t t = t_first;; ++t) {
         const bool have_tile = t <= t_last;
         if (have_tile) {
@@ -569,10 +579,110 @@
     if (c == 0) flags[g] = fl_c[k] ? 1 : 0;
 }
 
+constexpr int kFixupRecBytes = 4 * kFQ * kFQ * 8;
+template <typename T, int LPS>
+__global__ __launch_bounds__(64) void fixup_marked_kernel(const T* const* __restrict__ cols, int p, const int64_t* __restrict__ offsets,
+                                                          SolveRegDev sp, const int32_t* __restrict__ list, unsigned* __restrict__ state,
+                                                          unsigned* __restrict__ mark_host_flag, T* __restrict__ coeffs,
+                                                          uint8_t* __restrict__ flags) {
+    constexpr int SPW = 64 / LPS;
+    extern __shared__ __attribute__((aligned(16))) char smem[];
+    const int lane = threadIdx.x & 63;
+    const unsigned count = __hip_atomic_load(&state[0], __ATOMIC_RELAXED, __HIP_MEMORY_SCOPE_AGENT);
+    if (count == 0u) return;
+    {
+        char* wl = smem;
+        double* rec = reinterpret_cast<double*>(wl);
+        T* recs = reinterpret_cast<T*>(smem + kWaveLds);
+        const int pp = sp.pp, q = p + 2;
+        const int sub = lane / LPS, j = lane % LPS;
+        ColPtrs<T> cp;
+        fetch_col_ptrs<T, false>(cols, p, cp);
+        const unsigned nbatch = (count + (unsigned)SPW - 1u) / (unsigned)SPW;
+        for (unsigned b = blockIdx.x; b < nbatch; b += gridDim.x) {
+            const unsigned k0 = b * (unsigned)SPW;
+            const int nk = (int)min((unsigned)SPW, count - k0);
+            for (int s = 0; s < nk; ++s) {
+                const int64_t gg = (int64_t)list[k0 + s];
+                const int64_t r0 = offsets[gg], rend = offsets[gg + 1], ng = rend - r0;
+                WaveAcc acc;
+                zero_acc(acc);
+                int64_t done = 0;
+                do {
+                    GroupRegs<T> regs;
+                    load_group_tile<T>(cp, p, r0 + done, rend, lane, regs);
+                    PDS_WAVE_LDS_SYNC();
+                    store_group_lds<T>(wl, p, lane, regs);
+                    const int64_t left = ng - done;
+                    const int rows = (int)(left < 128 ? left : 128);
+                    consume_tile<T, false>(wl, lane, (rows + 3) >> 2, acc);
+                    done += 128;
+                } while (done < ng);
+                PDS_WAVE_LDS_SYNC();
+                wave_record<T>(acc, lane, rec);
+                PDS_WAVE_LDS_SYNC();
+                T* o = recs + s * (q * q);
+                for (int idx = lane; idx < q * q; idx += 64) {
+                    int i = idx % q, jj = idx / q;
+                    if (i > jj) { int tmp = i; i = jj; jj = tmp; }
+                    double v;
+                    if (jj < p) v = rec[kPartD + i + 16 * jj];
+                    else if (jj == p) v = (i < p) ? rec[kPartCS + i] : (double)ng;
+                    else v = (i < p) ? rec[kPartXY + i] : (i == p ? rec[kPartYS] : rec[kPartYY]);
+                    o[idx] = (T)v;
+                }
+                PDS_WAVE_LDS_SYNC();
+            }
+            const bool live = sub < nk;
+            const T* M = recs + (live ? sub : 0) * (q * q);
+            auto elem = [&](int i, int k) __attribute__((always_inline)) -> double { return (double)M[i + k * q]; };
+            const bool colv = j < pp;
+            double dj = colv ? elem(j, j) : 1.0;
+            const bool lam = sp.lambda > 0.0 && colv && (j < p || sp.lambda_on_bias);
+            if (lam) dj += sp.lambda;
+            bool is_null = false;
+            int pj = j;
+            double zj = 0.0;
+            double a[LPS], bb[LPS];
+#pragma unroll
+            for (int i = 0; i < LPS; ++i) {
+                a[i] = (colv && i < pp) ? elem(i, j) : 0.0;
+                if (lam && i == j) a[i] += sp.lambda;
+                bb[i] = (i < pp) ? elem(i, p + 1) : 0.0;
+            }
+            solve_core<LPS>(a, bb, dj, j, lane, sp, is_null, pj, zj);
+            const int64_t sys = live ? (int64_t)list[k0 + sub] : 0;
+            if (live && colv) coeffs[sys * (int64_t)pp + pj] = is_null ? (T)__builtin_nan("") : (T)zj;
+            if (live && j == 0) flags[sys] = is_null ? 1 : 0;
+            PDS_WAVE_LDS_SYNC();
+        }
+    }
+    if (lane == 0) {
+        const unsigned gone = __hip_atomic_fetch_add(&state[1], 1u, __ATOMIC_ACQ_REL, __HIP_MEMORY_SCOPE_AGENT);
+        if (gone == gridDim.x - 1u) {
+            __hip_atomic_store(&state[0], 0u, __ATOMIC_RELAXED, __HIP_MEMORY_SCOPE_AGENT);
+            __hip_atomic_store(&state[1], 0u, __ATOMIC_RELAXED, __HIP_MEMORY_SCOPE_AGENT);
+            __hip_atomic_store(mark_host_flag, 0u, __ATOMIC_RELAXED, __HIP_MEMORY_SCOPE_SYSTEM);
+        }
+    }
+}
+
+template <typename T, int LPS>
+static int launch_fixup_lps(pds_ctx* ctx, const DeviceCols<T>& dc, int n_feat, const int64_t* d_offsets, const SolveRegDev& sq,
+                            const int32_t* d_list, unsigned* d_state, unsigned* d_host, T* d_coeffs, uint8_t* d_flags) {
+    const unsigned nb = (unsigned)std::max(1, std::min(ctx->num_cus, 1024));
+    hipLaunchKernelGGL((fixup_marked_kernel<T, LPS>), dim3(nb), dim3(64), (size_t)kWaveLds + kFixupRecBytes, ctx->stream, dc.d_ptrs, n_feat,
+                       d_offsets, sq, d_list, d_state, d_host, d_coeffs, d_flags);
+    PDS_HIP_CHECK(hipGetLastError());
+    return PDS_OK;
+}
+
 template <typename T>
 int launch_grouped_fused(pds_ctx* ctx, const DeviceCols<T>& dc, int n_feat, int64_t n_rows, const int64_t* d_offsets,
                          int64_t n_groups, const SolveParams& sp, T* d_coeffs, uint8_t* d_flags, T* d_mom_scratch,
-                         int64_t scratch_groups) {
+                         int64_t scratch_groups, bool* stay_on_stream) {
+    const bool want_stream = stay_on_stream && *stay_on_stream;
+    if (stay_on_stream) *stay_on_stream = false;
     SolveRegDev sd;
     sd.p = sp.p;
     sd.bias = sp.add_bias ? 1 : 0;
@@ -591,21 +701,49 @@
     int32_t* d_list = nullptr;
     unsigned* d_count = nullptr;
     unsigned* d_host = nullptr;
+    const bool dev_fixup = want_stream && second_pass && sp.solver == PDS_SOLVER_QR && sd.pp <= 16;
     if (second_pass) {
         if (int rc0 = ensure_mark_state(ctx)) return rc0;
         d_list = reinterpret_cast<int32_t*>(ws_take(ctx, (size_t)n_groups * sizeof(int32_t)));
         if (!d_list) return fail(PDS_ERR_HIP, "workspace allocation failed");
         d_count = ctx->mark_count;
         d_host = ctx->mark_host_dev;
-        *ctx->mark_host = 0u;
-        if (ctx->mark_dirty) PDS_HIP_CHECK(hipMemsetAsync(d_count, 0, sizeof(unsigned), ctx->stream));
+        if (!dev_fixup && ctx->async_pending) {
+            PDS_HIP_CHECK(hipStreamSynchronize(ctx->stream));
+            ctx->async_pending = false;
+        }
+        if (!dev_fixup) *ctx->mark_host = 0u;
+        if (ctx->mark_dirty) PDS_HIP_CHECK(hipMemsetAsync(d_count, 0, 2 * sizeof(unsigned), ctx->stream));
         ctx->mark_dirty = true;
     }
     int rc;
     if (sd.p <= 4) rc = launch_stream_lps<T, 4>(ctx, dc, n_feat, d_offsets, n_groups, n_rows, sd, chol, d_coeffs, d_flags, d_list, d_count, d_host);
     else if (sd.p <= 8) rc = launch_stream_lps<T, 8>(ctx, dc, n_feat, d_offsets, n_groups, n_rows, sd, chol, d_coeffs, d_flags, d_list, d_count, d_host);
     else rc = launch_stream_lps<T, 16>(ctx, dc, n_feat, d_offsets, n_groups, n_rows, sd, chol, d_coeffs, d_flags, d_list, d_count, d_host);
-    if (rc || !second_pass) return rc;
+    if (rc) return rc;
+    if (!second_pass) {
+        if (stay_on_stream) *stay_on_stream = want_stream;
+        return PDS_OK;
+    }
+    if (dev_fixup) {
+        SolveRegDev sq;
+        sq.p = sp.p;
+        sq.bias = sd.bias;
+        sq.pp = sd.pp;
+        sq.lambda_on_bias = sp.lambda_on_bias;
+        sq.lambda = sp.lambda;
+        sq.gate_on = sd.gate_on;
+        sq.ln_tol = sd.ln_tol;
+        sq.inv_tol = sd.inv_tol;
+        int rcf;
+        if (sq.pp <= 4) rcf = launch_fixup_lps<T, 4>(ctx, dc, n_feat, d_offsets, sq, d_list, d_count, d_host, d_coeffs, d_flags);
+        else if (sq.pp <= 8) rcf = launch_fixup_lps<T, 8>(ctx, dc, n_feat, d_offsets, sq, d_list, d_count, d_host, d_coeffs, d_flags);
+        else rcf = launch_fixup_lps<T, 16>(ctx, dc, n_feat, d_offsets, sq, d_list, d_count, d_host, d_coeffs, d_flags);
+        if (rcf) return rcf;
+        ctx->mark_dirty = false;
+        *stay_on_stream = true;
+        return PDS_OK;
+    }
     PDS_HIP_CHECK(hipStreamSynchronize(ctx->stream));
     if (__atomic_load_n(ctx->mark_host, __ATOMIC_ACQUIRE) == 0u) {
         ctx->mark_dirty = false;
@@ -644,17 +782,19 @@
 #endif
 
 #ifdef PDS_WAVE_STAMPS
+extern "C" int pds_debug_wave_stamp_words(void) { return kStampWords; }
 extern "C" int pds_debug_wave_stamps(unsigned long long* out, int max_waves) {
     const int n = std::min(std::min(g_stamp_grid, kStampWaves), max_waves);
     if (n <= 0) return 0;
-    if (hipMemcpyFromSymbol(out, HIP_SYMBOL(g_wave_stamps), (size_t)n * 4 * sizeof(unsigned long long)) != hipSuccess) return -1;
+    if (hipDeviceSynchronize() != hipSuccess) return -1;
+    if (hipMemcpyFromSymbol(out, HIP_SYMBOL(g_wave_stamps), (size_t)n * kStampWords * sizeof(unsigned long long)) != hipSuccess) return -1;
     return n;
 }
 #endif
 
 template int launch_grouped_fused<double>(pds_ctx*, const DeviceCols<double>&, int, int64_t, const int64_t*, int64_t,
-                                          const SolveParams&, double*, uint8_t*, double*, int64_t);
+                                          const SolveParams&, double*, uint8_t*, double*, int64_t, bool*);
 template int launch_grouped_fused<float>(pds_ctx*, const DeviceCols<float>&, int, int64_t, const int64_t*, int64_t,
-                                         const SolveParams&, float*, uint8_t*, float*, int64_t);
-
-}
+                                         const SolveParams&, float*, uint8_t*, float*, int64_t, bool*);
+
+}
diff --git a/polars_ds_extension_amd/lstsq.py b/polars_ds_extension_amd/lstsq.py
--- a/polars_ds_extension_amd/lstsq.py
+++ b/polars_ds_extension_amd/lstsq.py
@@ -67,7 +67,8 @@
 
 class Context:
 
-    def __init__(self, device: int = 0, stream=None):
+    def __init__(self, device: int = 0, stream=None, follow_torch: bool = True):
+        self._follow_torch = bool(follow_torch)
         self._lib = _lib.load()
         self._h = C.c_void_p()
         _lib.check(self._lib.pds_ctx_create(int(device), C.byref(self._h)))
@@ -81,6 +82,8 @@
         self._stream_raw = int(raw) if raw else 0
 
     def follow_torch_stream(self, device) -> None:
+        if not getattr(self, "_follow_torch", True):
+            return
         import torch
 
         raw = int(torch.cuda.current_stream(device).cuda_stream)
@@ -98,6 +101,14 @@
         v = C.c_longlong(0)
         _lib.check(self._lib.pds_ctx_get_option(self._h, str(name).encode(), C.byref(v)))
         return int(v.value)
+
+    def last_return_async(self) -> bool:
+        return bool(self._lib.pds_debug_last_return_async(self._h))
+
+    def mark_state(self) -> tuple:
+        w = (C.c_uint * 2)()
+        _lib.check(self._lib.pds_debug_mark_state(self._h, w))
+        return int(w[0]), int(w[1])
 
     @property
     def num_cus(self) -> int:
```

New measurement: 422.0 million regressions/s (median of 6 runs). +1.8%, better.
